# SohirMaskey/raincast-gnn

Hardware: AMD Instinct MI355X
Metric: training graphs/s (24h_mixed GNN, full train step) (higher is better)
Workload: dtype f32 (split-bf16x3 GEMM products, fp32 accumulate); 1 GPU; cfg2: 24h_mixed, 32 graphs x 500 stations, k=10, 4 GINE layers, D=128; global_batch=32, graphs_per_gpu=32, nodes_per_gpu=16000, edges_per_gpu=176000, parallelism=dp1, hip_graph=True, station_order=locality, allreduce_in_graph=False, allreduce_overlap=False, head_fold=True

## Files before the change

include/gine_hip.h:

```cpp
#ifndef GINE_HIP_H_
#define GINE_HIP_H_

#include <stddef.h>
#include <stdint.h>

#ifdef __cplusplus
extern "C" {
#endif

#define GINE_ABI_VERSION 10

#define GINE_OK 0
#define GINE_ERR_INVALID 1
#define GINE_ERR_DIM 2
#define GINE_ERR_WORKSPACE 3
#define GINE_ERR_TOO_LARGE 4
#define GINE_ERR_HIP_BASE 1000

int gine_abi_version(void);
const char* gine_status_string(int status);

int gine_graph_workspace_bytes(int64_t num_nodes, int64_t num_edges, size_t* bytes);
int gine_graph_build(const int64_t* edge_index, const float* edge_attr, int64_t num_nodes,
                     int64_t num_edges, int32_t* in_rowptr, int32_t* in_src, float* in_attr,
                     int32_t* out_rowptr, int32_t* out_dst, float* out_attr, int32_t* d_error,
                     void* workspace, size_t workspace_bytes, void* stream);
int gine_graph_same_edges(const int64_t* edge_index_a, const int64_t* edge_index_b,
                          const float* edge_attr_a, const float* edge_attr_b, int64_t num_edges,
                          int32_t* differ, void* stream);
int gine_graph_build_ek(const int64_t* edge_index, const float* edge_attr, int64_t num_nodes,
                        int64_t num_edges, int32_t edge_dim, int32_t* in_rowptr,
                        int32_t* in_src, float* in_attr, int32_t* out_rowptr, int32_t* out_dst,
                        float* out_attr, int32_t* out_eid, int32_t* d_error, void* workspace,
                        size_t workspace_bytes, void* stream);
int gine_graph_same_edges_ek(const int64_t* edge_index_a, const int64_t* edge_index_b,
                             const float* edge_attr_a, const float* edge_attr_b,
                             int64_t num_edges, int32_t edge_dim, int32_t* differ, void* stream);
int gine_host_device_ptr(void* host_ptr, void** device_ptr);

#define GINE_MP_LIN_MULADD 2
int gine_mp_fwd(const float* x, const int32_t* in_rowptr, const int32_t* in_src,
                const float* in_attr, const float* lin_w, const float* lin_b, const float* eps,
                float* z, int64_t num_nodes, int32_t channels, int32_t flags, void* stream);

#define GINE_MP_BWD_SELF 1
int gine_mp_bwd_num_partials(int64_t num_nodes, int32_t channels, int32_t* num_partials);
int gine_mp_bwd(const float* dz, const float* x, const int32_t* out_rowptr,
                const int32_t* out_dst, const float* out_attr, const float* lin_w,
                const float* lin_b, const float* eps, const float* dres, float* dx,
                double* partials, int64_t num_nodes, int32_t channels, int32_t flags,
                void* stream);
int gine_mp_bwd_finalize(const double* partials, int32_t num_partials, int32_t channels,
                         float* dlin_w, float* dlin_b, float* deps, void* stream);
int gine_mp_bwd_side(const float* dz, const float* x, const int32_t* out_rowptr,
                     const int32_t* out_dst, const float* out_attr, const float* lin_w,
                     const float* lin_b, const float* eps, const float* dres, float* dx,
                     double* partials, int64_t num_nodes, int32_t channels, int32_t flags,
                     const float* wg_slab, int32_t wg_chunks, int32_t mlp_channels, float* dw1,
                     float* db1, float* dw2, float* db2, void* stream);

#define GINE_MP_MAX_EDGE_DIM 8
int gine_mp_fwd_ek(const float* x, const int32_t* in_rowptr, const int32_t* in_src,
                   const float* in_attr, const float* lin_w, const float* lin_b,
                   const float* eps, float* z, int64_t num_nodes, int64_t num_edges,
                   int32_t channels, int32_t edge_dim, void* stream);
int gine_mp_bwd_ek_num_partials(int64_t num_nodes, int32_t channels, int32_t edge_dim,
                                int32_t* num_partials);
int gine_mp_bwd_ek(const float* dz, const float* x, const int32_t* out_rowptr,
                   const int32_t* out_dst, const float* out_attr, const int32_t* out_eid,
                   const float* lin_w, const float* lin_b, const float* eps, const float* dres,
                   float* dx, float* dea, double* partials, int64_t num_nodes,
                   int64_t num_edges, int32_t channels, int32_t edge_dim, int32_t flags,
                   void* stream);
int gine_mp_bwd_ek_finalize(const double* partials, int32_t num_partials, int32_t channels,
                            int32_t edge_dim, float* dlin_w, float* dlin_b, float* deps,
                            void* stream);

#define GINE_WINDOW_LDS_BYTES (80 * 1024)
typedef struct gine_window_plan {
  const int32_t* tile_begin;
  const int32_t* win_lo;
  const int32_t* win_rows;
  int32_t num_tiles;
  int32_t slice_channels;
  int32_t max_rows, max_edges, max_nodes;
  const int16_t* slot;
  const int32_t* edge_begin;
} gine_window_plan;
int gine_graph_plan_windows(const int32_t* rowptr, const int32_t* nbr, int64_t num_nodes,
                            int32_t max_rows, int32_t max_nodes, int32_t max_edges,
                            int32_t* tile_begin, int32_t* win_lo, int32_t* win_rows,
                            int32_t* num_tiles, int32_t* maxima);
int gine_graph_plan_window_slots(const int32_t* rowptr, const int32_t* tile_begin,
                                 int32_t num_tiles, int16_t* slot);
int gine_graph_order_locality(const int32_t* rowptr, const int32_t* nbr, int64_t num_nodes,
                              int32_t* order);
int gine_mp_fwd_win(const float* x, const int32_t* in_rowptr, const int32_t* in_src,
                    const float* in_attr, const float* lin_w, const float* lin_b,
                    const float* eps, float* z, int64_t num_nodes, int32_t channels,
                    int32_t flags, const gine_window_plan* plan, void* stream);
int gine_mp_bwd_win(const float* dz, const float* x, const int32_t* out_rowptr,
                    const int32_t* out_dst, const float* out_attr, const float* lin_w,
                    const float* lin_b, const float* eps, const float* dres, float* dx,
                    double* partials, int64_t num_nodes, int32_t channels, int32_t flags,
                    const gine_window_plan* plan, void* stream);
int gine_mp_bwd_win_side(const float* dz, const float* x, const int32_t* out_rowptr,
                         const int32_t* out_dst, const float* out_attr, const float* lin_w,
                         const float* lin_b, const float* eps, const float* dres, float* dx,
                         double* partials, int64_t num_nodes, int32_t channels, int32_t flags,
                         const gine_window_plan* plan, const float* wg_slab, int32_t wg_chunks,
                         int32_t mlp_channels, float* dw1, float* db1, float* dw2, float* db2,
                         void* stream);
int gine_mp_bwd_win_mlp_wgrad(const float* dz, const float* x, const int32_t* out_rowptr,
                              const int32_t* out_dst, const float* out_attr,
                              const float* lin_w, const float* lin_b, const float* eps,
                              const float* dres, float* dx, double* partials,
                              int64_t num_nodes, int32_t channels, int32_t flags,
                              const gine_window_plan* plan, const float* dy, const float* y,
                              const uint8_t* mask, const float* a1, const float* bn_save,
                              const float* dbn, const float* coef, const float* z, float* slab,
                              int32_t epilogue, void* stream);
int gine_mp_bwd_win_finalize(const double* partials, int32_t num_tiles, int32_t channels,
                             int32_t slice_channels, float* dlin_w, float* dlin_b,
                             float* deps, void* stream);

#define GINE_GRAD_JOB_MP 1
#define GINE_GRAD_JOB_SLAB 2
#define GINE_GRAD_MAX_JOBS 12
typedef struct gine_grad_job {
  int32_t kind;
  int32_t rows;
  int32_t channels;
  int32_t eps_cols;
  int32_t nz;
  int32_t pad_;
  const void* src;
  int64_t cstride, zstride;
  int64_t per[4];
  int64_t wsize[4];
  float bscale[4];
  float* w[4];
  float* b[4];
} gine_grad_job;
int gine_grad_finalize_batch(const gine_grad_job* jobs, int32_t num_jobs, void* stream);
int gine_head_bwd_grad_job(int64_t num_nodes, int32_t channels, int32_t kind, const float* slab,
                           float* dw, float* db, gine_grad_job* job);
int gine_chain_wgrad_grad_job(int64_t num_nodes, int32_t hidden, int32_t in_features,
                              const float* slab, float bias_scale, float* dwp2, float* dbp2,
                              float* dwr0, float* dbr0, float* dwr1, float* dbr1, float* dwdr,
                              float* dbdr, gine_grad_job* job);
int gine_deepset_bwd_grad_job(int64_t num_nodes, int32_t in_features, int32_t hidden,
                              const float* slab, float* dw1, float* db1, gine_grad_job* job);

#define GINE_EPI_NONE 0
#define GINE_EPI_RELU 1
#define GINE_EPI_RESIDUAL_RELU 2

int gine_mlp_num_partials(int64_t num_nodes, int32_t channels, int32_t* num_partials);
int gine_mlp_fwd1(const float* z, const float* w1, const float* b1, float* a1, double* partials,
                  int64_t num_nodes, int32_t channels, void* stream);
int gine_bn_fwd_finalize(const double* partials, int32_t num_partials, const float* gamma,
                         const float* beta, float* running_mean, float* running_var,
                         int64_t* num_batches_tracked, float* bn_save, int64_t num_nodes,
                         int32_t channels, float momentum, float bn_eps, int32_t training,
                         int32_t update_running, void* stream);
int gine_mlp_fwd2(const float* a1, const float* bn_save, const float* w2, const float* b2,
                  const float* x, float* y, uint8_t* mask, int64_t num_nodes, int32_t channels,
                  int32_t epilogue, void* stream);

#define GINE_MP_FUSED_MAX_DEGREE 32
int gine_mp_fwd_mlp1(const float* x, const int32_t* in_rowptr, const int32_t* in_src,
                     const float* in_attr, const float* lin_w, const float* lin_b,
                     const float* eps, const float* w1, const float* b1, float* z, float* a1,
                     double* partials, int64_t num_nodes, int32_t channels,
                     int32_t max_in_degree, int32_t flags, void* stream);

int gine_bn_acc_words(int32_t channels, int64_t* words);
int gine_bn_acc_barrier_failures_index(int32_t channels, int64_t* index);
int gine_mlp_bwd2_acc(const float* dy, const float* y, const uint8_t* mask, const float* a1,
                      const float* bn_save, const float* w2, float* dbn, double* partials,
                      int64_t* bn_acc, int64_t num_nodes, int32_t channels, int32_t epilogue,
                      void* stream);
int gine_mlp_bwd1_bn(const float* dbn, const float* a1, const float* bn_save, int64_t* bn_acc,
                     const float* gamma, float* dgamma, float* dbeta, float* coef,
                     const float* w1, float* dz, int64_t num_nodes, int32_t channels,
                     void* stream);
int gine_mlp_bwd_layer_ok(int64_t num_nodes, int32_t channels, int32_t* ok);
int gine_mlp_bwd_layer(const float* dy, const float* y, const uint8_t* mask, const float* a1,
                       const float* bn_save, const float* w2, float* dbn, int64_t* bn_acc,
                       const float* gamma, float* dgamma, float* dbeta, float* coef,
                       const float* w1, float* dz, int64_t num_nodes, int32_t channels,
                       int32_t epilogue, void* stream);
int gine_testing_bwd_layer_extra_workgroups(int32_t extra);
int gine_mlp_fwd1_acc(const float* z, const float* w1, const float* b1, float* a1,
                      double* partials, int64_t* bn_acc, int64_t num_nodes, int32_t channels,
                      void* stream);
int gine_mp_fwd_mlp1_acc(const float* x, const int32_t* in_rowptr, const int32_t* in_src,
                         const float* in_attr, const float* lin_w, const float* lin_b,
                         const float* eps, const float* w1, const float* b1, float* z,
                         float* a1, double* partials, int64_t* bn_acc, int64_t num_nodes,
                         int32_t channels, int32_t max_in_degree, int32_t flags, void* stream);
int gine_mp_fwd_layer_ok(int64_t num_nodes, int32_t channels, int32_t max_in_degree, int32_t* ok);
int gine_testing_layer_extra_workgroups(int32_t extra);
int gine_testing_sum_32(const float* in, float* out, int32_t waves, int32_t mode, void* stream);
typedef struct gine_layer_head {
  const float* weight;
  const float* bias;
  float* raw;
  float* pred;
  const float* y_target;
  uint32_t* count_parts;
  int32_t kind;
} gine_layer_head;
int gine_mp_fwd_layer(const float* x, const int32_t* in_rowptr, const int32_t* in_src,
                      const float* in_attr, const float* lin_w, const float* lin_b,
                      const float* eps, const float* w1, const float* b1, float* z, float* a1,
                      int64_t* bn_acc, const float* gamma, const float* beta,
                      float* running_mean, float* running_var, int64_t* num_batches_tracked,
                      float* bn_save, float momentum, float bn_eps, int32_t update_running,
                      const float* w2, const float* b2, float* y, uint8_t* mask,
                      int64_t num_nodes, int32_t channels, int32_t max_in_degree, int32_t flags,
                      int32_t epilogue, const int32_t* tile_windows, int32_t window_rows,
                      const gine_layer_head* head, void* stream);
int gine_mp_fwd_layer_eval(const float* x, const int32_t* in_rowptr, const int32_t* in_src,
                           const float* in_attr, const float* lin_w, const float* lin_b,
                           const float* eps, const float* w1, const float* b1,
                           const float* gamma, const float* beta, const float* running_mean,
                           const float* running_var, float bn_eps, const float* w2,
                           const float* b2, float* y, int64_t num_nodes, int32_t channels,
                           int32_t max_in_degree, int32_t flags, int32_t epilogue,
                           const gine_layer_head* head, int32_t max_workgroups, void* stream);
int gine_mp_fwd_layer_eval_deep(const float* x, const int32_t* in_rowptr, const int32_t* in_src,
                                const float* in_attr, const float* lin_w, const float* lin_b,
                                const float* eps, const float* w1, const float* b1,
                                const float* gamma, const float* beta,
                                const float* running_mean, const float* running_var,
                                float bn_eps, const float* w2, const float* b2, float* y,
                                int64_t num_nodes, int32_t channels, int32_t max_in_degree,
                                int32_t flags, int32_t epilogue, const gine_layer_head* head,
                                int32_t max_workgroups, void* stream);
int gine_graph_plan_layer_windows(const int32_t* in_rowptr, const int32_t* in_src,
                                  int64_t num_nodes, int32_t* tile_windows, int32_t* maxima,
                                  void* stream);
int gine_mp_fwd_layer_windows_fit(int32_t window_rows, int32_t max_in_degree, int32_t* ok);
int gine_mlp_fwd2_bn(const float* a1, int64_t* bn_acc, const float* gamma, const float* beta,
                     float* running_mean, float* running_var, int64_t* num_batches_tracked,
                     float* bn_save, float momentum, float bn_eps, int32_t update_running,
                     const float* w2, const float* b2, const float* x, float* y,
                     uint8_t* mask, int64_t num_nodes, int32_t channels, int32_t epilogue,
                     void* stream);

int gine_mlp_bwd2(const float* dy, const float* y, const uint8_t* mask, const float* a1,
                  const float* bn_save, const float* w2, float* dbn, double* partials,
                  int64_t num_nodes, int32_t channels, int32_t epilogue, void* stream);
int gine_bn_bwd_finalize(const double* partials, int32_t num_partials, const float* gamma,
                         const float* bn_save, float* dgamma, float* dbeta, float* coef,
                         int64_t num_nodes, int32_t channels, int32_t training, void* stream);
int gine_mlp_bwd1(const float* dbn, const float* a1, const float* bn_save, const float* coef,
                  const float* w1, float* dz, int64_t num_nodes, int32_t channels,
                  void* stream);
int gine_mlp_wgrad_num_chunks(int64_t num_nodes, int32_t channels, int32_t* num_chunks);
int gine_mlp_wgrad(const float* dy, const float* y, const uint8_t* mask, const float* a1,
                   const float* bn_save, const float* dbn, const float* coef, const float* z,
                   float* slab, float* dw1, float* db1, float* dw2, float* db2,
                   int64_t num_nodes, int32_t channels, int32_t epilogue, void* stream);

int gine_mlp_bwd1_wgrad(const float* dy, const float* y, const uint8_t* mask, const float* a1,
                        const float* bn_save, const float* dbn, const float* coef,
                        const float* z, const float* w1, float* dz, float* slab, float* dw1,
                        float* db1, float* dw2, float* db2, int64_t num_nodes,
                        int32_t channels, int32_t epilogue, void* stream);

int gine_adamw_step(float* param, const float* grad, float* exp_avg, float* exp_avg_sq,
                    float* step, int64_t n, float lr, float beta1, float beta2, float eps,
                    float weight_decay, void* stream);
int gine_adamw_state_floats(int64_t* floats);

#define GINE_LOSS_NORMAL 0
#define GINE_LOSS_MIXED_NORMAL 1
#define GINE_LOSS_MIXED 2
#define GINE_LOSS_MIXED_U 3
int gine_crps_num_partials(int64_t num_nodes, int32_t* num_partials);
int gine_crps_fwd(const float* pred, const float* y, int64_t num_nodes, int32_t kind, double u,
                  double xi, double c, double t, double* dpred, double* partials,
                  double* loss_out, double* count_out, uint32_t* ticket, void* stream);
int gine_crps_bwd(const double* dpred, const double* count, const double* gloss,
                  int64_t num_nodes, int32_t kind, float* grad_pred, void* stream);
#define GINE_COUNT_PARTS 64
int gine_count_valid(const float* y, int64_t num_nodes, uint32_t* count_parts, void* stream);
int gine_crps_fwd_grad(const float* pred, const float* y, int64_t num_nodes, int32_t kind,
                       double u, double xi, double c, double t, double* dpred, double* partials,
                       double* loss_out, double* count_out, uint32_t* ticket,
                       const uint32_t* count_parts, float* grad_unit, void* stream);
int gine_crps_head_slab_floats(int64_t num_nodes, int32_t channels, int32_t kind,
                               size_t* floats);
int gine_crps_head_fwd_grad(const float* pred, const float* y, int64_t num_nodes, int32_t kind,
                            double u, double xi, double c, double t, double* dpred,
                            double* partials, double* loss_out, double* count_out,
                            uint32_t* ticket, const uint32_t* count_parts, float* grad_unit,
                            const float* raw, const float* h, const float* w, int32_t channels,
                            float* dh, float* head_slab, void* stream);
int gine_crps_head_grad_job(int64_t num_nodes, int32_t channels, int32_t kind,
                            const float* head_slab, float* dw, float* db, gine_grad_job* job);

#define GINE_FORECAST_UPPER 1
int gine_forecast_prob(const float* pred, int64_t num_nodes, int32_t kind, double u, double xi,
                       double c, const double* x, int32_t num_x, int32_t flags, double* out,
                       void* stream);
int gine_forecast_quantile(const float* pred, int64_t num_nodes, int32_t kind, double u,
                           double xi, double c, const double* level, int32_t num_levels,
                           int32_t flags, double* out, void* stream);
int gine_forecast_score_partials(int64_t num_nodes, int32_t num_x, size_t* count);
int gine_forecast_score(const float* pred, const float* y, int64_t num_nodes, int32_t kind,
                        double u, double xi, double c, const double* x, int32_t num_x,
                        double* crps_rows, double* pit_lo, double* pit_hi, double* brier,
                        double* valid, double* partials, uint32_t* ticket, void* stream);

int gine_linear_wgrad_num_chunks(int64_t rows, int32_t out_features, int32_t in_features,
                                 int32_t* num_chunks);
int gine_linear_wgrad(const float* dy, const float* x, int64_t rows, int32_t out_features,
                      int32_t in_features, float* slab, float* dw, float* db, float bias_scale,
                      void* stream);

int gine_deepset_mask_bytes(int64_t num_nodes, int32_t members, int32_t hidden, size_t* bytes);
int gine_deepset_mask_layout(int64_t num_nodes, int32_t hidden, int32_t* nodes_per_half);
int gine_deepset_fwd(const float* ens, const float* w1, const float* b1, float* r,
                     uint16_t* mask, int64_t num_nodes, int32_t members, int32_t in_features,
                     int32_t hidden, void* stream);
int gine_deepset_fwd_fold2(const float* ens, const float* w1, const float* b1, float* r,
                           uint16_t* mask, int64_t num_nodes, int32_t members,
                           int32_t in_features, int32_t hidden, const float* wr1,
                           const float* br1, const float* wdr, const float* bdr, float* wfold,
                           int32_t x_features, const float* wr0, const float* br0,
                           const float* wp2, const float* bp2, float* wfold2, void* stream);
int gine_deepset_bwd_num_partials(int64_t num_nodes, int32_t hidden, int32_t* num_partials);
int gine_deepset_bwd(const float* ens, const uint16_t* mask, const float* dr, float* slab,
                     float* dw1, float* db1, int64_t num_nodes, int32_t members,
                     int32_t in_features, int32_t hidden, void* stream);

int gine_head_fwd(const float* h, const float* w, const float* b, float* raw, float* pred,
                  int64_t num_nodes, int32_t channels, int32_t kind, void* stream);
int gine_head_fwd_count(const float* h, const float* w, const float* b, float* raw,
                        float* pred, int64_t num_nodes, int32_t channels, int32_t kind,
                        const float* y, uint32_t* count_parts, void* stream);
int gine_head_bwd_slab_floats(int64_t num_nodes, int32_t channels, int32_t kind,
                              size_t* floats);
int gine_head_bwd(const float* grad_pred, const float* raw, const float* h, const float* w,
                  float* dh, float* slab, float* dw, float* db, int64_t num_nodes,
                  int32_t channels, int32_t kind, void* stream);
int gine_head_bwd_reduce(const float* slab, float* dw, float* db, int64_t num_nodes,
                         int32_t channels, int32_t kind, void* stream);

int gine_chain_bwd_slab_floats(int64_t num_nodes, int32_t hidden, int32_t in_features,
                               size_t* floats);
int gine_chain_fwd_folded2(const float* r, const float* x, const float* wfold,
                           const float* wfold2, float* u, float* h0, int64_t num_nodes,
                           int32_t hidden, int32_t in_features, void* stream);
int gine_chain_bwd_folded2(const float* dh0, const float* u, const float* wfold,
                           const float* wfold2, float* dt, float* dr, int64_t num_nodes,
                           int32_t hidden, int32_t in_features, void* stream);
int gine_chain_wgrad_folded2(const float* dh0, const float* x, const float* r, const float* u,
                             const float* dt, float* slab, float* gfold, float* g2fold,
                             int64_t num_nodes, int32_t hidden, int32_t in_features,
                             void* stream);
int gine_chain_wgrad_folded2_grad_job(int64_t num_nodes, int32_t hidden, int32_t in_features,
                                      const float* slab, float* gfold, float* g2fold,
                                      gine_grad_job* job);
int gine_chain_unfold_grads2(const float* gfold, const float* wr1, const float* br1,
                             const float* wdr, float* dwdr, float* dbdr, float* dwr1,
                             float* dbr1, const float* g2fold, const float* wp2,
                             const float* bp2, const float* wr0, float* dwr0, float* dbr0,
                             float* dwp2, float* dbp2, float members, int32_t hidden,
                             int32_t in_features, void* stream);
int gine_chain_fwd(const float* r, const float* x, const float* wp2, const float* bp2,
                   float bias_scale, const float* wr0, const float* br0, const float* wr1,
                   const float* br1, const float* wdr, const float* bdr, float* s, float* u,
                   float* e, float* h0, int64_t num_nodes, int32_t hidden,
                   int32_t in_features, void* stream);
int gine_chain_bwd(const float* dh0, const float* x, const float* r, const float* s,
                   const float* u, const float* e, const float* wp2, const float* wr0,
                   const float* wr1, const float* wdr, float* de, float* dt, float* ds,
                   float* dr, float* slab, float* dwp2, float* dbp2, float bias_scale,
                   float* dwr0, float* dbr0, float* dwr1, float* dbr1, float* dwdr,
                   float* dbdr, int64_t num_nodes, int32_t hidden, int32_t in_features,
                   void* stream);
int gine_chain_wgrad(const float* dh0, const float* x, const float* r, const float* s,
                     const float* u, const float* e, const float* de, const float* dt,
                     const float* ds, float* slab, float* dwp2, float* dbp2, float bias_scale,
                     float* dwr0, float* dbr0, float* dwr1, float* dbr1, float* dwdr,
                     float* dbdr, int64_t num_nodes, int32_t hidden, int32_t in_features,
                     void* stream);


int gine_copy_f4(const void* src, void* dst, int64_t bytes, void* stream);
int gine_probe_chain(int32_t variant, int32_t reps, int32_t blocks, float* sink,
                     long long* ticks, void* stream);

#ifdef __cplusplus
}
#endif

#endif
```

raincast-gnn_amd/csrc/gine_chain.hip:

```cpp
#include "gine_common.hpp"
#include "gine_slab.hpp"
#include "gine_wgrad.hpp"
#include "gine_chainfold.hpp"

#include <algorithm>

namespace gine {
namespace {

typedef float floatx16 __attribute__((ext_vector_type(16)));

constexpr int kRowTile = 32;

#ifdef GINE_CHAIN_PROFILE
__device__ long long g_chain_prof[1024][16];
#define CHAIN_MARK(i)                                                          \
  do {                                                                         \
    if (threadIdx.x == 0 && blockIdx.x < 1024)                                 \
      g_chain_prof[blockIdx.x][i] = (long long)__builtin_amdgcn_s_memtime();  \
  } while (0)
#define CHAIN_RT(i)                                                            \
  do {                                                                         \
    if (threadIdx.x == 0 && blockIdx.x < 1024)                                 \
      g_chain_prof[blockIdx.x][i] = (long long)__builtin_amdgcn_s_memrealtime(); \
  } while (0)
#else
#define CHAIN_MARK(i) do {} while (0)
#define CHAIN_RT(i) do {} while (0)
#endif

enum ChainKind { CH_F2D, CH_B2D, CH_F1, CH_F2, CH_B1, CH_B2 };

struct ChainArgs {
  const float* in;
  const float* x;
  const float* aux;
  const float* w1;
  const float* b1;
  const float* w2;
  const float* b2;
  float* out1;
  float* out2;
  float bias1_scale;
  int F;
  const float* w3;
  float* out3;
  const float* b3;
};

__device__ __forceinline__ floatx16 zero16() {
  floatx16 v;
#pragma unroll
  for (int i = 0; i < 16; ++i) v[i] = 0.f;
  return v;
}

template <int K>
__device__ __forceinline__ floatx16 tile_mma(const float* sA, int lda, const float (&bf)[K / 2],
                                             int c32, int h) {
  constexpr int KS = K / 2;
  floatx16 acc = zero16();
  const float* arow = sA + c32 * lda + h * KS;
#pragma unroll
  for (int q = 0; q < KS / 4; ++q) {
    const float4 a4 = *reinterpret_cast<const float4*>(&arow[4 * q]);
    acc = __builtin_amdgcn_mfma_f32_32x32x2f32(a4.x, bf[4 * q], acc, 0, 0, 0);
    acc = __builtin_amdgcn_mfma_f32_32x32x2f32(a4.y, bf[4 * q + 1], acc, 0, 0, 0);
    acc = __builtin_amdgcn_mfma_f32_32x32x2f32(a4.z, bf[4 * q + 2], acc, 0, 0, 0);
    acc = __builtin_amdgcn_mfma_f32_32x32x2f32(a4.w, bf[4 * q + 3], acc, 0, 0, 0);
  }
  return acc;
}

template <int K>
__device__ __forceinline__ void frag_t(float (&bf)[K / 2], const float* W, int ldw, int col,
                                       int h) {
  constexpr int KS = K / 2;
#pragma unroll
  for (int s = 0; s < KS; ++s) bf[s] = W[(size_t)col * ldw + h * KS + s];
}
template <int K>
__device__ __forceinline__ void frag_t4(float (&bf)[K / 2], const float* W, int ldw, int col,
                                        int h) {
  constexpr int KS = K / 2;
  const float4* row = reinterpret_cast<const float4*>(W + (size_t)col * ldw + h * KS);
#pragma unroll
  for (int s = 0; s < KS / 4; ++s) {
    const float4 v = row[s];
    bf[4 * s] = v.x;
    bf[4 * s + 1] = v.y;
    bf[4 * s + 2] = v.z;
    bf[4 * s + 3] = v.w;
  }
}
template <int K>
__device__ __forceinline__ void frag_n(float (&bf)[K / 2], const float* W, int ldw, int coff,
                                       int col, int h) {
  constexpr int KS = K / 2;
#pragma unroll
  for (int s = 0; s < KS; ++s) bf[s] = W[(size_t)(h * KS + s) * ldw + coff + col];
}
template <int FP, int D>
__device__ __forceinline__ void frag_dimred(float (&bf)[(FP + D) / 2], const float* W, int F,
                                            int col, int h) {
  constexpr int KS = (FP + D) / 2;
  const int ldw = F + D;
#pragma unroll
  for (int s = 0; s < KS; ++s) {
    const int k = h * KS + s;
    const int c = k < F ? k : (k < FP ? 0 : k - FP + F);
    const float v = W[(size_t)col * ldw + c];
    bf[s] = (k >= F && k < FP) ? 0.f : v;
  }
}
template <int FP, int D>
__device__ __forceinline__ void frag_dimred_t(float (&bf)[(FP + D) / 2], const float* WT, int F,
                                              int col, int h) {
  constexpr int KS = (FP + D) / 2;
#pragma unroll
  for (int s = 0; s < KS; ++s) {
    const int k = h * KS + s;
    const int c = k < F ? k : (k < FP ? 0 : k - FP + F);
    const float v = WT[(size_t)c * D + col];
    bf[s] = (k >= F && k < FP) ? 0.f : v;
  }
}

struct TileRange {
  int first, end, step;
};
__device__ __forceinline__ TileRange tile_range(int num_tiles, int nb) {
  const int xcd = blockIdx.x % kNumXcd, pos = blockIdx.x / kNumXcd;
  const int here = nb / kNumXcd + (xcd < nb % kNumXcd ? 1 : 0);
  const int span = (num_tiles + kNumXcd - 1) / kNumXcd;
  const int b = xcd * span;
  return TileRange{b + pos, min(num_tiles, b + span), here};
}

template <int D, int FP, int KIND>
__global__ __launch_bounds__(2 * D) void k_chain(ChainArgs a, int64_t N, int num_tiles) {
  constexpr int NT = 2 * D;
  constexpr int D4 = D / 4;
  constexpr int LDA = D + 4;
  constexpr bool kDimRed = KIND == CH_F2;
  constexpr int K2 = kDimRed ? FP + D : D;
  constexpr int LDB = K2 + 4;
  constexpr int BOFF = kDimRed ? FP : 0;
  constexpr int ITEMS = kRowTile * D4 / NT;
  constexpr int RSTEP = NT / D4;
  constexpr int XITEMS = (kRowTile * FP + NT - 1) / NT;
  constexpr bool kF2D = KIND == CH_F2D, kB2D = KIND == CH_B2D;
  constexpr bool kMask = KIND == CH_B1 || kB2D;
  constexpr bool kX = kDimRed || kF2D;
  constexpr int LDC = FP + D + 4;
  __shared__ __attribute__((aligned(16))) float sA[kRowTile * LDA];
  __shared__ __attribute__((aligned(16))) float sB[kF2D ? 4 : kRowTile * LDB];
  __shared__ __attribute__((aligned(16))) float sC[kF2D ? kRowTile * LDC : 4];

  const int wave = threadIdx.x / kWave, lane = threadIdx.x % kWave;
  const int h = lane >> 5, c32 = lane & 31;
  const int col = wave * 32 + c32;
  const int q_me = threadIdx.x % D4, r_me = threadIdx.x / D4;
  CHAIN_RT(11);
  CHAIN_MARK(0);
  const int nb = gridDim.x;

  float bf1[D / 2], bf2[K2 / 2];
  const bool w16 =
      ((reinterpret_cast<uintptr_t>(a.w1) | reinterpret_cast<uintptr_t>(a.w2)) & 15) == 0;
  if constexpr (KIND == CH_F1) {
    if (w16) {
      frag_t4<D>(bf1, a.w1, D, col, h);
      frag_t4<D>(bf2, a.w2, D, col, h);
    } else {
      frag_t<D>(bf1, a.w1, D, col, h);
      frag_t<D>(bf2, a.w2, D, col, h);
    }
  } else if constexpr (kF2D) {
    if (w16) frag_t4<D>(bf1, a.w1, D, col, h);
    else frag_t<D>(bf1, a.w1, D, col, h);
  } else if constexpr (KIND == CH_F2) {
    frag_t<D>(bf1, a.w1, D, col, h);
  } else if constexpr (kMask) {
    frag_n<D>(bf1, a.w1, a.F + D, a.F, col, h);
  } else if constexpr (KIND == CH_B2) {
    frag_n<D>(bf1, a.w1, D, 0, col, h);
  }
  if constexpr (KIND == CH_F2) {
    frag_dimred<FP, D>(bf2, a.w2, a.F, col, h);
  } else if constexpr (KIND == CH_B1 || KIND == CH_B2 || kB2D) {
    frag_n<D>(bf2, a.w2, D, 0, col, h);
  }
  float bf3[kF2D ? (FP + D) / 2 : 1];
  if constexpr (kF2D) frag_dimred_t<FP, D>(bf3, a.w3, a.F, col, h);
  float bias1 = 0.f, bias2 = 0.f, bias3 = 0.f;
  if constexpr (KIND == CH_F1 || KIND == CH_F2 || kF2D) bias1 = a.b1[col] * a.bias1_scale;
  if constexpr (KIND == CH_F1 || kDimRed) bias2 = a.b2[col];
  if constexpr (kF2D) bias3 = a.b3[col];
  CHAIN_MARK(1);

  auto load_tile = [&](int tile, float4 (&raw)[ITEMS], float (&xr)[XITEMS]) {
    const int64_t n0 = (int64_t)tile * kRowTile;
#pragma unroll
    for (int i = 0; i < ITEMS; ++i) {
      int64_t n = n0 + r_me + i * RSTEP;
      n = n < N ? n : N - 1;
      raw[i] = reinterpret_cast<const float4*>(a.in + n * D)[q_me];
    }
    if constexpr (kX) {
#pragma unroll
      for (int i = 0; i < XITEMS; ++i) {
        const int idx = threadIdx.x + i * NT;
        const int r = idx / FP, c = idx % FP;
        int64_t n = n0 + r;
        n = n < N ? n : N - 1;
        xr[i] = a.x[n * a.F + min(c, a.F - 1)];
      }
    }
  };

  const TileRange tr = tile_range(num_tiles, nb);
  float4 raw[ITEMS];
  float xr[XITEMS];
  if (tr.first < tr.end) load_tile(tr.first, raw, xr);
  int kt = 0;
  for (int tile = tr.first; tile < tr.end; tile += tr.step, ++kt) {
    const int64_t n0 = (int64_t)tile * kRowTile;
    float ep[16];
    if constexpr (kMask) {
#pragma unroll
      for (int r = 0; r < 16; ++r) {
        int64_t n = n0 + (r & 3) + 8 * (r >> 2) + 4 * h;
        n = n < N ? n : N - 1;
        ep[r] = a.aux[n * D + col];
      }
    }
    __syncthreads();
#pragma unroll
    for (int i = 0; i < ITEMS; ++i) {
      const int r = r_me + i * RSTEP;
      const float4 v = (n0 + r < N) ? raw[i] : f4_zero();
      float* dst = &sA[r * LDA + 4 * q_me];
      *reinterpret_cast<float4*>(dst) = v;
    }
    if constexpr (kX) {
      float* sx = kF2D ? sC : sB;
      constexpr int LDX = kF2D ? LDC : LDB;
#pragma unroll
      for (int i = 0; i < XITEMS; ++i) {
        const int idx = threadIdx.x + i * NT;
        if (idx < kRowTile * FP) sx[(idx / FP) * LDX + idx % FP] = idx % FP < a.F ? xr[i] : 0.f;
      }
    }
    __syncthreads();
    if (kt < 2) CHAIN_MARK(2 + 4 * kt);
    if (tile + tr.step < tr.end) load_tile(tile + tr.step, raw, xr);

    floatx16 acc;
    acc = tile_mma<D>(sA, LDA, bf1, c32, h);
#pragma unroll
    for (int r = 0; r < 16; ++r) {
      const int rr = (r & 3) + 8 * (r >> 2) + 4 * h;
      const int64_t n = n0 + rr;
      float v = acc[r] + bias1;
      if constexpr (kB2D) v = ep[r] > 0.f ? acc[r] : 0.f;
      if constexpr (kF2D) {
        v = relu_nan(v);
        sC[rr * LDC + FP + col] = v;
      } else {
        sB[rr * LDB + BOFF + col] = v;
      }
      if (n < N) a.out1[n * D + col] = v;
    }
    if (kt < 2) CHAIN_MARK(3 + 4 * kt);
    __syncthreads();
    if (kt < 2) CHAIN_MARK(4 + 4 * kt);

    if constexpr (!kF2D) {
      acc = tile_mma<K2>(sB, LDB, bf2, c32, h);
#pragma unroll
      for (int r = 0; r < 16; ++r) {
        const int rr = (r & 3) + 8 * (r >> 2) + 4 * h;
        const int64_t n = n0 + rr;
        float v = acc[r] + bias2;
        if constexpr (KIND == CH_F1) v = relu_nan(v);
        if constexpr (KIND == CH_B1) v = ep[r] > 0.f ? v : 0.f;
        if (n < N) a.out2[n * D + col] = v;
      }
    } else {
      acc = tile_mma<FP + D>(sC, LDC, bf3, c32, h);
#pragma unroll
      for (int r = 0; r < 16; ++r) {
        const int64_t n = n0 + (r & 3) + 8 * (r >> 2) + 4 * h;
        if (n < N) a.out3[n * D + col] = acc[r] + bias3;
      }
    }
    if (kt < 2) CHAIN_MARK(5 + 4 * kt);
  }
  CHAIN_MARK(10);
  CHAIN_RT(12);
}

inline int chain_grid(int64_t N) {
  const int64_t tiles = ceil_div(N, kRowTile);
  return (int)std::max<int64_t>(1, std::min<int64_t>(tiles, kNumCu));
}

template <int D, int FP, int KIND>
int launch_chain(const ChainArgs& a, int64_t N, hipStream_t s) {
  const int tiles = (int)ceil_div(N, kRowTile);
  hipLaunchKernelGGL((k_chain<D, FP, KIND>), dim3(chain_grid(N)), dim3(2 * D), 0, s, a, N,
                     tiles);
  GINE_LAUNCH_STATUS();
  return GINE_OK;
}

template <int NZ>
struct ChainWgradSrc {
  static constexpr int kZ = NZ;
  const float* p[NZ];
  const float* q[NZ];
  const float* x;
  int D, F;
  struct Raw {
    float4 v;
  };
  struct Col {
    float keep[4];
  };
  template <int Z> __device__ int i_dim(int) const { return Z == 0 ? F + D : D; }
  template <int Z> __device__ Col p_col(int) const { return Col{{1.f, 1.f, 1.f, 1.f}}; }
  template <int Z> __device__ Col q_col(int q4) const {
    Col c{{1.f, 1.f, 1.f, 1.f}};
    if constexpr (Z == 0) {
#pragma unroll
      for (int j = 0; j < 4; ++j) c.keep[j] = 4 * q4 + j < F + D ? 1.f : 0.f;
    }
    return c;
  }
  template <int Z> __device__ Raw p_load(int64_t n, int q4) const {
    return Raw{reinterpret_cast<const float4*>(p[Z] + n * D)[q4]};
  }
  template <int Z> __device__ Raw q_load(int64_t n, int q4) const {
    if constexpr (Z == 0) {
      const int I = F + D;
      float v[4];
#pragma unroll
      for (int j = 0; j < 4; ++j) {
        const int c = min(4 * q4 + j, I - 1);
        const float* src = c < F ? x + n * F + c : q[0] + n * D + (c - F);
        v[j] = *src;
      }
      return Raw{make_float4(v[0], v[1], v[2], v[3])};
    } else {
      return Raw{reinterpret_cast<const float4*>(q[Z] + n * D)[q4]};
    }
  }
  template <int Z> __device__ float4 p_xform(const Raw& r, const Col&) const { return r.v; }
  template <int Z> __device__ float4 q_xform(const Raw& r, const Col& c) const {
    if constexpr (Z == 0)
      return make_float4(c.keep[0] != 0.f ? r.v.x : 0.f, c.keep[1] != 0.f ? r.v.y : 0.f,
                         c.keep[2] != 0.f ? r.v.z : 0.f, c.keep[3] != 0.f ? r.v.w : 0.f);
    return r.v;
  }
};

struct ChainWgradOut {
  float* w[4];
  float* b[4];
  int D, F;
  float bscale3;
  __device__ void operator()(int z, int64_t e, double v) const {
    const int64_t I = z == 0 ? F + D : D;
    const int64_t ws = (int64_t)D * I;
    if (e < ws) {
      w[z][e] = (float)v;
    } else if (e < ws + D && b[z] != nullptr) {
      b[z][e - ws] = (float)(z == 3 ? v * (double)bscale3 : v);
    }
  }
};

struct ChainWgradShape {
  WgPlan plan;
  int nz;
  int tiles;
  size_t per;
  size_t zstride() const { return per * plan.chunks; }
  size_t slab_floats() const { return nz * zstride(); }
};
inline ChainWgradShape chain_wgrad_shape(int64_t N, int D, int F, int nz) {
  const int to = (int)ceil_div(D, 64);
  ChainWgradShape s;
  s.nz = nz;
  s.tiles = to * (int)ceil_div(F + D, kWgTI) + (nz - 1) * to * (int)ceil_div(D, kWgTI);
  s.plan = wg_plan(N, D, F + D, nz, 64, s.tiles);
  s.per = (size_t)D * (D + F) + D;
  return s;
}

void chain_slab_job(const ChainWgradShape& sh, int D, int F, const float* slab, float bscale3,
                    float* const* w, float* const* b, gine_grad_job* job) {
  *job = gine_grad_job{};
  job->kind = GINE_GRAD_JOB_SLAB;
  job->src = slab;
  job->rows = sh.plan.chunks;
  job->cstride = (int64_t)sh.per;
  job->zstride = (int64_t)sh.zstride();
  job->nz = sh.nz;
  for (int z = 0; z < sh.nz; ++z) {
    const int64_t ws = (int64_t)D * (z == 0 ? F + D : D);
    job->per[z] = ws + D;
    job->wsize[z] = ws;
    job->w[z] = w[z];
    job->b[z] = b[z];
    job->bscale[z] = z == 3 ? bscale3 : 1.0f;
  }
}

inline bool chain_dims_ok(int D, int F) { return (D == 64 || D == 128) && F >= 1 && F <= 64; }

#define GINE_CHAIN_DISPATCH(D_, F_, CALL)                          \
  do {                                                             \
    if ((D_) == 64) {                                              \
      if ((F_) <= 40) { CALL(64, 40); } else { CALL(64, 64); }     \
    } else {                                                       \
      if ((F_) <= 40) { CALL(128, 40); } else { CALL(128, 64); }   \
    }                                                              \
  } while (0)

struct UnfoldJob {
  const float *gf, *w1, *b1, *wdr;
  float *dwdr, *dbdr, *dw1, *db1;
  int F;
  float bscale;
};

template <int D>
__global__ __launch_bounds__(2 * D) void k_chain_unfold(UnfoldJob j0, UnfoldJob j1) {
  constexpr int NT = 2 * D, LDA = D + 4, T = D / 32, TT = T * T;
  constexpr int SI = 32 * D / NT, XI = 32 * 64 / NT;
  __shared__ __attribute__((aligned(16))) float sA[32 * LDA];
  __shared__ float sR[T * kSR];
  __shared__ float svec[D];
  const bool second = (int)blockIdx.x >= 2 * TT;
  const UnfoldJob J{second ? j1.gf : j0.gf,     second ? j1.w1 : j0.w1,
                    second ? j1.b1 : j0.b1,     second ? j1.wdr : j0.wdr,
                    second ? j1.dwdr : j0.dwdr, second ? j1.dbdr : j0.dbdr,
                    second ? j1.dw1 : j0.dw1,   second ? j1.db1 : j0.db1,
                    second ? j1.F : j0.F,       second ? j1.bscale : j0.bscale};
  const int blk = (int)blockIdx.x - (second ? 2 * TT : 0);
  const float* __restrict__ gf = J.gf;
  const int F = J.F;
  const int LW = F + D;
  const float* g = gf + (size_t)D * LW;
  const int w = threadIdx.x / kWave, lane = threadIdx.x % kWave;
  const int h = lane >> 5, c32 = lane & 31;
  const bool e_cols = blk < TT;
  const int t = e_cols ? blk : blk - TT;
  const int r0 = 32 * (t / T), c0 = 32 * (t % T);
  float bf[16], st[SI];
  if (e_cols) {
#pragma unroll
    for (int s = 0; s < 16; ++s) bf[s] = J.w1[(size_t)(c0 + c32) * D + w * 32 + h * 16 + s];
#pragma unroll
    for (int i = 0; i < SI; ++i) {
      const int idx = threadIdx.x + i * NT;
      st[i] = gf[(size_t)(r0 + idx / D) * LW + F + idx % D];
    }
    if (c0 == 0) {
      if (F > 0) {
        float xv[XI];
#pragma unroll
        for (int i = 0; i < XI; ++i) {
          const int idx = min(threadIdx.x + i * NT, 32 * F - 1);
          xv[i] = gf[(size_t)(r0 + idx / F) * LW + idx % F];
        }
#pragma unroll
        for (int i = 0; i < XI; ++i) {
          const int idx = threadIdx.x + i * NT;
          if (idx < 32 * F) J.dwdr[(size_t)(r0 + idx / F) * LW + idx % F] = xv[i];
        }
      }
      if (threadIdx.x < 32 && J.dbdr != nullptr) J.dbdr[r0 + threadIdx.x] = g[r0 + threadIdx.x];
    }
#pragma unroll
    for (int i = 0; i < SI; ++i) {
      const int idx = threadIdx.x + i * NT;
      sA[(idx / D) * LDA + idx % D] = st[i];
    }
  } else {
#pragma unroll
    for (int s = 0; s < 16; ++s)
      bf[s] = gf[(size_t)(w * 32 + h * 16 + s) * LW + F + c0 + c32];
#pragma unroll
    for (int i = 0; i < SI; ++i) {
      const int idx = threadIdx.x + i * NT;
      st[i] = J.wdr[(size_t)(idx / 32) * LW + F + r0 + idx % 32];
    }
    const float gv = threadIdx.x < D ? g[threadIdx.x] : 0.f;
#pragma unroll
    for (int i = 0; i < SI; ++i) {
      const int idx = threadIdx.x + i * NT;
      sA[(idx % 32) * LDA + idx / 32] = st[i];
    }
    if (threadIdx.x < D) svec[threadIdx.x] = gv;
  }
  __syncthreads();
  ksplit_tile<D>(sA, bf, sR, c32, h);
  if (!e_cols && c0 == 0) {
    const float v = rows_dot<D>(sA, svec);
    constexpr int TPR = NT / 32;
    if (threadIdx.x % TPR == 0 && J.db1 != nullptr) J.db1[r0 + threadIdx.x / TPR] = v * J.bscale;
  }
  __syncthreads();
#pragma unroll
  for (int i = 0; i < 1024 / NT; ++i) {
    const int o = threadIdx.x + i * NT, rr = o / 32, cc = o % 32;
    const float v = ksplit_sum<D>(sR, rr, cc);
    if (e_cols)
      J.dwdr[(size_t)(r0 + rr) * LW + F + c0 + cc] =
          fmaf(g[r0 + rr], J.b1[c0 + cc] * J.bscale, v);
    else
      J.dw1[(size_t)(r0 + rr) * D + c0 + cc] = v;
  }
}

int launch_unfold(int D, const UnfoldJob& j0, const UnfoldJob& j1, hipStream_t st) {
  if (D == 64)
    hipLaunchKernelGGL((k_chain_unfold<64>), dim3(2 * 2 * 4), dim3(128), 0, st, j0, j1);
  else
    hipLaunchKernelGGL((k_chain_unfold<128>), dim3(2 * 2 * 16), dim3(256), 0, st, j0, j1);
  GINE_LAUNCH_STATUS();
  return GINE_OK;
}

}
}

using namespace gine;

extern "C" int gine_chain_bwd_slab_floats(int64_t num_nodes, int32_t hidden,
                                          int32_t in_features, size_t* floats) {
  if (!floats || num_nodes < 0) return GINE_ERR_INVALID;
  if (!chain_dims_ok(hidden, in_features)) return GINE_ERR_DIM;
  *floats = std::max(chain_wgrad_shape(num_nodes, hidden, in_features, 2).slab_floats(),
                     chain_wgrad_shape(num_nodes, hidden, in_features, 4).slab_floats());
  return GINE_OK;
}

extern "C" int gine_chain_fwd_folded2(const float* r, const float* x, const float* wfold,
                                      const float* wfold2, float* u, float* h0,
                                      int64_t num_nodes, int32_t hidden, int32_t in_features,
                                      void* stream) {
  if (!chain_dims_ok(hidden, in_features)) return GINE_ERR_DIM;
  if (num_nodes < 0) return GINE_ERR_INVALID;
  if (num_nodes >= (int64_t(1) << 31)) return GINE_ERR_TOO_LARGE;
  if (num_nodes == 0) return GINE_OK;
  if (!r || !x || !wfold || !wfold2 || !u || !h0) return GINE_ERR_INVALID;
  hipStream_t st = as_stream(stream);
  const int D = hidden, F = in_features;
  const float* bfold = wfold + (size_t)D * (F + D);
  ChainArgs f{r, x, nullptr, wfold2, wfold2 + (size_t)D * D, nullptr, nullptr, u, nullptr,
              1.f, F};
  f.w3 = bfold + D;
  f.b3 = bfold;
  f.out3 = h0;
  int rc = GINE_OK;
#define CALL_F(DD, FF) rc = launch_chain<DD, FF, CH_F2D>(f, num_nodes, st)
  GINE_CHAIN_DISPATCH(D, F, CALL_F);
#undef CALL_F
  return rc;
}

extern "C" int gine_chain_bwd_folded2(const float* dh0, const float* u, const float* wfold,
                                      const float* wfold2, float* dt, float* dr,
                                      int64_t num_nodes, int32_t hidden, int32_t in_features,
                                      void* stream) {
  if (!chain_dims_ok(hidden, in_features)) return GINE_ERR_DIM;
  if (num_nodes <= 0) return GINE_ERR_INVALID;
  if (num_nodes >= (int64_t(1) << 31)) return GINE_ERR_TOO_LARGE;
  if (!dh0 || !u || !wfold || !wfold2 || !dt || !dr) return GINE_ERR_INVALID;
  hipStream_t st = as_stream(stream);
  const int F = in_features;
  const ChainArgs b{dh0, nullptr, u, wfold, nullptr, wfold2, nullptr, dt, dr, 1.f, F};
  int rc = GINE_OK;
#define CALL_B(DD, FF) rc = launch_chain<DD, FF, CH_B2D>(b, num_nodes, st)
  GINE_CHAIN_DISPATCH(hidden, F, CALL_B);
#undef CALL_B
  return rc;
}

extern "C" int gine_chain_wgrad_folded2(const float* dh0, const float* x, const float* r,
                                        const float* u, const float* dt, float* slab,
                                        float* gfold, float* g2fold, int64_t num_nodes,
                                        int32_t hidden, int32_t in_features, void* stream) {
  if (!chain_dims_ok(hidden, in_features)) return GINE_ERR_DIM;
  if (num_nodes <= 0) return GINE_ERR_INVALID;
  if (!dh0 || !x || !r || !u || !dt || !slab) return GINE_ERR_INVALID;
  const bool reduce = gfold || g2fold;
  if (reduce && (!gfold || !g2fold)) return GINE_ERR_INVALID;
  hipStream_t st = as_stream(stream);
  const int D = hidden, F = in_features;
  const ChainWgradShape sh = chain_wgrad_shape(num_nodes, D, F, 2);
  const ChainWgradSrc<2> src{{dh0, dt}, {u, r}, x, D, F};
  int rc = launch_wgrad_engine<64>(src, num_nodes, D, D + F, sh.tiles, sh.plan, sh.zstride(),
                                   sh.per, slab, st);
  if (rc != GINE_OK || !reduce) return rc;
  return launch_slab_sum(slab, sh.plan.chunks, (int64_t)sh.per, sh.per, sh.zstride(), sh.nz,
                         ChainWgradOut{{gfold, g2fold, nullptr, nullptr},
                                       {gfold + (size_t)D * (F + D), g2fold + (size_t)D * D,
                                        nullptr, nullptr},
                                       D, F, 1.f},
                         st);
}

extern "C" int gine_chain_wgrad_folded2_grad_job(int64_t num_nodes, int32_t hidden,
                                                 int32_t in_features, const float* slab,
                                                 float* gfold, float* g2fold,
                                                 gine_grad_job* job) {
  if (!chain_dims_ok(hidden, in_features)) return GINE_ERR_DIM;
  if (num_nodes <= 0 || !slab || !gfold || !g2fold || !job) return GINE_ERR_INVALID;
  const int D = hidden, F = in_features;
  float* w[2] = {gfold, g2fold};
  float* b[2] = {gfold + (size_t)D * (D + F), g2fold + (size_t)D * D};
  chain_slab_job(chain_wgrad_shape(num_nodes, D, F, 2), D, F, slab, 1.f, w, b, job);
  return GINE_OK;
}

extern "C" int gine_chain_unfold_grads2(const float* gfold, const float* wr1, const float* br1,
                                        const float* wdr, float* dwdr, float* dbdr, float* dwr1,
                                        float* dbr1, const float* g2fold, const float* wp2,
                                        const float* bp2, const float* wr0, float* dwr0,
                                        float* dbr0, float* dwp2, float* dbp2, float members,
                                        int32_t hidden, int32_t in_features, void* stream) {
  if (!chain_dims_ok(hidden, in_features)) return GINE_ERR_DIM;
  if (!gfold || !wr1 || !br1 || !wdr || !dwdr || !dwr1) return GINE_ERR_INVALID;
  if (!g2fold || !wp2 || !bp2 || !wr0 || !dwr0 || !dwp2) return GINE_ERR_INVALID;
  return launch_unfold(hidden,
                       UnfoldJob{gfold, wr1, br1, wdr, dwdr, dbdr, dwr1, dbr1, in_features, 1.f},
                       UnfoldJob{g2fold, wp2, bp2, wr0, dwr0, dbr0, dwp2, dbp2, 0, members},
                       as_stream(stream));
}

extern "C" int gine_chain_fwd(const float* r, const float* x, const float* wp2, const float* bp2,
                              float bias_scale, const float* wr0, const float* br0,
                              const float* wr1, const float* br1, const float* wdr,
                              const float* bdr, float* s, float* u, float* e, float* h0,
                              int64_t num_nodes, int32_t hidden, int32_t in_features,
                              void* stream) {
  if (!chain_dims_ok(hidden, in_features)) return GINE_ERR_DIM;
  if (num_nodes < 0) return GINE_ERR_INVALID;
  if (num_nodes >= (int64_t(1) << 31)) return GINE_ERR_TOO_LARGE;
  if (num_nodes == 0) return GINE_OK;
  if (!r || !x || !wp2 || !bp2 || !wr0 || !br0 || !wr1 || !br1 || !wdr || !bdr || !s || !u ||
      !e || !h0)
    return GINE_ERR_INVALID;
  hipStream_t st = as_stream(stream);
  const ChainArgs f1{r, nullptr, nullptr, wp2, bp2, wr0, br0, s, u, bias_scale, in_features};
  const ChainArgs f2{u, x, nullptr, wr1, br1, wdr, bdr, e, h0, 1.f, in_features};
  int rc = GINE_OK;
#define CALL_F(DD, FF)                                                  \
  rc = launch_chain<DD, FF, CH_F1>(f1, num_nodes, st);                  \
  if (rc == GINE_OK) rc = launch_chain<DD, FF, CH_F2>(f2, num_nodes, st)
  GINE_CHAIN_DISPATCH(hidden, in_features, CALL_F);
#undef CALL_F
  return rc;
}

extern "C" int gine_chain_bwd(const float* dh0, const float* x, const float* r, const float* s,
                              const float* u, const float* e, const float* wp2,
                              const float* wr0, const float* wr1, const float* wdr, float* de,
                              float* dt, float* ds, float* dr, float* slab, float* dwp2,
                              float* dbp2, float bias_scale, float* dwr0, float* dbr0,
                              float* dwr1, float* dbr1, float* dwdr, float* dbdr,
                              int64_t num_nodes, int32_t hidden, int32_t in_features,
                              void* stream) {
  if (!chain_dims_ok(hidden, in_features)) return GINE_ERR_DIM;
  if (num_nodes <= 0) return GINE_ERR_INVALID;
  if (num_nodes >= (int64_t(1) << 31)) return GINE_ERR_TOO_LARGE;
  if (!dh0 || !x || !r || !s || !u || !e || !wp2 || !wr0 || !wr1 || !wdr || !de || !dt ||
      !ds || !dr)
    return GINE_ERR_INVALID;
  if (slab && (!dwp2 || !dwr0 || !dwr1 || !dwdr)) return GINE_ERR_INVALID;
  hipStream_t st = as_stream(stream);
  const int D = hidden, F = in_features;
  const ChainArgs b1{dh0, nullptr, u, wdr, nullptr, wr1, nullptr, de, dt, 1.f, F};
  const ChainArgs b2{dt, nullptr, nullptr, wr0, nullptr, wp2, nullptr, ds, dr, 1.f, F};
  int rc = GINE_OK;
#define CALL_B(DD, FF)                                                  \
  rc = launch_chain<DD, FF, CH_B1>(b1, num_nodes, st);                  \
  if (rc == GINE_OK) rc = launch_chain<DD, FF, CH_B2>(b2, num_nodes, st)
  GINE_CHAIN_DISPATCH(D, F, CALL_B);
#undef CALL_B
  if (rc != GINE_OK || !slab) return rc;
  return gine_chain_wgrad(dh0, x, r, s, u, e, de, dt, ds, slab, dwp2, dbp2, bias_scale, dwr0,
                          dbr0, dwr1, dbr1, dwdr, dbdr, num_nodes, hidden, in_features, stream);
}

extern "C" int gine_chain_wgrad(const float* dh0, const float* x, const float* r,
                                const float* s, const float* u, const float* e,
                                const float* de, const float* dt, const float* ds, float* slab,
                                float* dwp2, float* dbp2, float bias_scale, float* dwr0,
                                float* dbr0, float* dwr1, float* dbr1, float* dwdr, float* dbdr,
                                int64_t num_nodes, int32_t hidden, int32_t in_features,
                                void* stream) {
  if (!chain_dims_ok(hidden, in_features)) return GINE_ERR_DIM;
  if (num_nodes <= 0) return GINE_ERR_INVALID;
  if (!dh0 || !x || !r || !s || !u || !e || !de || !dt || !ds || !slab) return GINE_ERR_INVALID;
  const bool reduce = dwp2 || dwr0 || dwr1 || dwdr;
  if (reduce && (!dwp2 || !dwr0 || !dwr1 || !dwdr)) return GINE_ERR_INVALID;
  hipStream_t st = as_stream(stream);
  const int D = hidden, F = in_features;
  const ChainWgradShape sh = chain_wgrad_shape(num_nodes, D, F, 4);
  const ChainWgradSrc<4> src{{dh0, de, dt, ds}, {e, u, s, r}, x, D, F};
  int rc = launch_wgrad_engine<64>(src, num_nodes, D, D + F, sh.tiles, sh.plan, sh.zstride(),
                                   sh.per, slab, st);
  if (rc != GINE_OK || !reduce) return rc;
  return launch_slab_sum(slab, sh.plan.chunks, (int64_t)sh.per, sh.per, sh.zstride(), sh.nz,
                         ChainWgradOut{{dwdr, dwr1, dwr0, dwp2}, {dbdr, dbr1, dbr0, dbp2}, D,
                                       F, bias_scale},
                         st);
}

extern "C" int gine_chain_wgrad_grad_job(int64_t num_nodes, int32_t hidden, int32_t in_features,
                                         const float* slab, float bias_scale, float* dwp2,
                                         float* dbp2, float* dwr0, float* dbr0, float* dwr1,
                                         float* dbr1, float* dwdr, float* dbdr,
                                         gine_grad_job* job) {
  if (!chain_dims_ok(hidden, in_features)) return GINE_ERR_DIM;
  if (num_nodes <= 0 || !slab || !dwp2 || !dwr0 || !dwr1 || !dwdr || !job)
    return GINE_ERR_INVALID;
  float* w[4] = {dwdr, dwr1, dwr0, dwp2};
  float* b[4] = {dbdr, dbr1, dbr0, dbp2};
  chain_slab_job(chain_wgrad_shape(num_nodes, hidden, in_features, 4), hidden, in_features,
                 slab, bias_scale, w, b, job);
  return GINE_OK;
}

#ifdef GINE_CHAIN_PROFILE
extern "C" int gine_debug_chain_prof(long long* out) {
  GINE_RETURN_IF_HIP(hipDeviceSynchronize());
  GINE_RETURN_IF_HIP(hipMemcpyFromSymbol(out, HIP_SYMBOL(g_chain_prof), sizeof(g_chain_prof)));
  return GINE_OK;
}
#endif
```

raincast-gnn_amd/csrc/gine_deepset.hip:

```cpp
#include "gine_common.hpp"
#include "gine_chainfold.hpp"
#include "gine_bf16x3.hpp"

#include <algorithm>

namespace gine {
namespace {

typedef float floatx16 __attribute__((ext_vector_type(16)));

__host__ __device__ constexpr int tiles_per_group(int G, int M) { return (G * M + 15) / 16; }

#ifndef GINE_DS_BF16X3
#define GINE_DS_BF16X3 1
#endif
template <int KP>
struct DsImg {
  static constexpr int KX = (KP + 15) / 16 * 16;
  static constexpr int RS = KX + 8;
  static constexpr int PLANE = 32 * RS;
  static constexpr int FLOATS = 3 * PLANE / 2;
};
template <int KI>
struct DsBwdImg {
  static_assert(KI == 32 || KI == 64, "feature tiles");
  static constexpr int RS = 40;
  static constexpr int PLANE = KI * RS;
  static constexpr int FLOATS = 3 * PLANE / 2;
};
constexpr int ds_bwd_ki(int KP) { return KP <= 32 ? 32 : 64; }
template <int KP, bool X3, int KI>
constexpr int stager_ld() {
  if constexpr (!X3) return KP + 4;
  else if constexpr (KI == 0) return DsImg<KP>::RS;
  else return DsBwdImg<KI>::RS;
}
template <int KP, bool X3, int KI>
constexpr int stager_plane() {
  if constexpr (!X3) return 0;
  else if constexpr (KI == 0) return DsImg<KP>::PLANE;
  else return DsBwdImg<KI>::PLANE;
}

#ifdef GINE_DS_PROFILE
__device__ long long g_ds_prof[4096];
__device__ int g_ds_prof_n;
#define DS_MARK(tag)                                                          \
  do {                                                                        \
    if (blockIdx.x == 0 && threadIdx.x == 0 && g_ds_prof_n < 2040) {          \
      g_ds_prof[2 * g_ds_prof_n] = (tag);                                     \
      g_ds_prof[2 * g_ds_prof_n + 1] = (long long)__builtin_amdgcn_s_memtime(); \
      ++g_ds_prof_n;                                                          \
    }                                                                         \
  } while (0)
#else
#define DS_MARK(tag) do {} while (0)
#endif

__device__ __forceinline__ floatx16 zero16() {
  floatx16 v;
#pragma unroll
  for (int i = 0; i < 16; ++i) v[i] = 0.f;
  return v;
}

__device__ __forceinline__ int staged_row(int i) {
  return 16 * ((i >> 2) & 1) + (i & 3) + 4 * (i >> 3);
}

#ifndef GINE_DS_BRANCHLESS
#define GINE_DS_BRANCHLESS 3
#endif
template <int NT, int KP, bool PAD, bool X3 = false, int KI = 0, bool BWD = false>
struct Stager {
  static constexpr int PER = (32 * KP + NT - 1) / NT;
  static constexpr int LD = stager_ld<KP, X3, KI>();
  static constexpr int kPlane = stager_plane<KP, X3, KI>();
  static constexpr bool kBranchless = (GINE_DS_BRANCHLESS & (BWD ? 1 : 2)) != 0;
  __device__ static int dummy_slot() {
    const int r = threadIdx.x & 31, u = threadIdx.x >> 5;
    if constexpr (X3 && KI != 0) return r * LD + 32 + (u & 7);
    else if constexpr (X3) return r * LD + DsImg<KP>::KX + (u & 7);
    else return r * LD + KP + (u & 3);
  }
  int src[PER];
  int row[PER];
  int dst[PER];
  uint32_t jrow[PAD ? PER : 1];
  __device__ __forceinline__ void init(int F, int M, int G) {
#pragma unroll
    for (int i = 0; i < PER; ++i) {
      const int e = threadIdx.x + i * NT;
      const int c = e >= 16 * F ? 1 : 0;
      const int off = e - c * 16 * F;
      const int j = off / F, f = off - j * F;
      const bool has = e < 32 * F;
      src[i] = has ? c * G * M * F + off : 0;
      row[i] = has ? c * G * M + j : 0x7fffffff;
      if constexpr (X3 && KI != 0)
        dst[i] = has ? f * LD + (16 * c + j) : (kBranchless ? dummy_slot() : -1);
      else
        dst[i] = has ? (16 * c + j) * LD + f : (kBranchless ? dummy_slot() : -1);
      if constexpr (PAD) jrow[i] = has ? (uint32_t)j : 0u;
    }
  }
  __device__ __forceinline__ uint32_t load(float (&v)[PER], const float* __restrict__ ens,
                                           int64_t row0, int64_t rows_total, int F,
                                           int half_lim) const {
    const int64_t d = rows_total - row0;
    const int lim = d <= 0 ? 0 : (d > 0x7fffffff ? 0x7fffffff : (int)d);
    const float* __restrict__ base = lim > 0 ? ens + row0 * F : ens;
    uint32_t ok = 0;
#pragma unroll
    for (int i = 0; i < PER; ++i) {
      bool in = row[i] < lim;
      if constexpr (PAD) in = in && (int)jrow[i] < half_lim;
      const int off = in ? src[i] : 0;
#ifdef GINE_BOUNDS_CHECK
      const int64_t a = (base - ens) + off;
      if (a < 0 || a >= rows_total * F) {
        printf("GINE_BOUNDS_CHECK deepset Stager::load: block %d thread %d reads ens[%lld] "
               "outside [0, %lld)\n", (int)blockIdx.x, (int)threadIdx.x, (long long)a,
               (long long)(rows_total * F));
        __builtin_trap();
      }
#endif
      v[i] = base[off];
      ok |= (in ? 1u : 0u) << i;
    }
    return ok;
  }
  __device__ __forceinline__ void store(float* s_e, const float (&v)[PER], uint32_t ok) const {
    if constexpr (X3) {
      constexpr int PL = kPlane;
      uint16_t* img = reinterpret_cast<uint16_t*>(s_e);
#pragma unroll
      for (int i = 0; i < PER; i += 2) {
        const int i1 = i + 1 < PER ? i + 1 : i;
        const float a = ((ok >> i) & 1u) ? v[i] : 0.f;
        const float b = ((ok >> i1) & 1u) ? v[i1] : 0.f;
        uint32_t ph, pm, pl;
        split2(a, b, ph, pm, pl);
        if (kBranchless || dst[i] >= 0) {
          img[dst[i]] = (uint16_t)ph;
          img[PL + dst[i]] = (uint16_t)pm;
          img[2 * PL + dst[i]] = (uint16_t)pl;
        }
        if (i + 1 < PER && (kBranchless || dst[i1] >= 0)) {
          img[dst[i1]] = (uint16_t)(ph >> 16);
          img[PL + dst[i1]] = (uint16_t)(pm >> 16);
          img[2 * PL + dst[i1]] = (uint16_t)(pl >> 16);
        }
      }
    } else {
#pragma unroll
      for (int i = 0; i < PER; ++i)
        if (kBranchless || dst[i] >= 0) s_e[dst[i]] = ((ok >> i) & 1u) ? v[i] : 0.f;
    }
  }
};

template <int KP>
__device__ __forceinline__ void zero_pad(float* s_e, int F) {
  constexpr int LD = KP + 4;
  for (int i = threadIdx.x; i < 32 * (LD - F); i += blockDim.x) {
    const int r = i / (LD - F), c = F + i % (LD - F);
    s_e[r * LD + c] = 0.f;
  }
}
template <int KP>
__device__ __forceinline__ void zero_pad_x3(float* s_e, int F) {
  using I = DsImg<KP>;
  uint16_t* img = reinterpret_cast<uint16_t*>(s_e);
  const int w = I::RS - F;
  for (int i = threadIdx.x; i < 3 * 32 * w; i += blockDim.x) {
    const int pr = i / w, c = F + i % w;
    img[pr * I::RS + c] = 0;
  }
}

template <int KP>
__device__ __forceinline__ floatx16 pre_tile(const float* s_e, const float (&bf)[KP / 2],
                                             int c32, int h) {
  constexpr int LD = KP + 4;
  constexpr int KS = KP / 2;
  floatx16 acc = zero16();
  const float* arow = s_e + staged_row(c32) * LD + h * KS;
#pragma unroll
  for (int q = 0; q < KS / 4; ++q) {
    const float4 a4 = *reinterpret_cast<const float4*>(arow + 4 * q);
    acc = __builtin_amdgcn_mfma_f32_32x32x2f32(a4.x, bf[4 * q], acc, 0, 0, 0);
    acc = __builtin_amdgcn_mfma_f32_32x32x2f32(a4.y, bf[4 * q + 1], acc, 0, 0, 0);
    acc = __builtin_amdgcn_mfma_f32_32x32x2f32(a4.z, bf[4 * q + 2], acc, 0, 0, 0);
    acc = __builtin_amdgcn_mfma_f32_32x32x2f32(a4.w, bf[4 * q + 3], acc, 0, 0, 0);
  }
  return acc;
}

template <int KP>
__device__ __forceinline__ floatx16 pre_tile_x3(const float* s_e,
                                                const Bf16x3 (&wb)[DsImg<KP>::KX / 16],
                                                int c32, int h) {
  using I = DsImg<KP>;
  const uint16_t* img = reinterpret_cast<const uint16_t*>(s_e) + staged_row(c32) * I::RS + 8 * h;
  floatx16 acc = zero16();
#pragma unroll
  for (int b = 0; b < I::KX / 16; ++b) {
    Bf16x3 a;
    a.h = *reinterpret_cast<const bf16x8_t*>(img + 16 * b);
    a.m = *reinterpret_cast<const bf16x8_t*>(img + I::PLANE + 16 * b);
    a.l = *reinterpret_cast<const bf16x8_t*>(img + 2 * I::PLANE + 16 * b);
    acc = mfma_bf16x3(a, wb[b], acc);
  }
  return acc;
}
template <int KP>
__device__ __forceinline__ void load_b_x3(const float* __restrict__ w1, int col, int h, int F,
                                          Bf16x3 (&wb)[DsImg<KP>::KX / 16]) {
#pragma unroll
  for (int b = 0; b < DsImg<KP>::KX / 16; ++b) {
    float v[8];
#pragma unroll
    for (int j = 0; j < 8; ++j) {
      const int k = 16 * b + 8 * h + j;
      v[j] = k < F ? w1[(size_t)col * F + k] : 0.f;
    }
    wb[b] = split8(make_float4(v[0], v[1], v[2], v[3]), make_float4(v[4], v[5], v[6], v[7]));
  }
}
template <int KP>
__device__ __noinline__ floatx16 pre_tile_mem(const float* __restrict__ ens,
                                              const float* __restrict__ w1, int64_t row0,
                                              int64_t rows_total, int GM, int half_lim, int F,
                                              int col, int c32, int h) {
  constexpr int KS = KP / 2;
  const int tr = staged_row(c32), c = tr >> 4, j = tr & 15;
  const int64_t grow = row0 + (int64_t)c * GM + j;
  const bool valid = grow < rows_total && j < half_lim;
  floatx16 acc = zero16();
#pragma unroll 1
  for (int s = 0; s < KS; ++s) {
    const int k = h * KS + s;
    const float a = (valid && k < F) ? ens[grow * F + k] : 0.f;
    const float b = k < F ? w1[(size_t)col * F + k] : 0.f;
    acc = __builtin_amdgcn_mfma_f32_32x32x2f32(a, b, acc, 0, 0, 0);
  }
  return acc;
}

template <int KP>
__device__ __forceinline__ void load_b(const float* __restrict__ w1, int col, int h, int F,
                                       float (&bf)[KP / 2]) {
  constexpr int KS = KP / 2;
#pragma unroll
  for (int s = 0; s < KS; ++s) {
    const int k = h * KS + s;
    bf[s] = k < F ? w1[(size_t)col * F + k] : 0.f;
  }
}

struct Groups {
  int first, step, end;
  __device__ __forceinline__ Groups(int num_groups, int nb, int b = (int)blockIdx.x) {
    const int xcd = b % kNumXcd, pos = b / kNumXcd;
    const int q = nb / kNumXcd, rm = nb % kNumXcd;
    const int here = q + (xcd < rm ? 1 : 0);
    const int before = xcd * q + min(xcd, rm);
    const int lo = (int)((int64_t)num_groups * before / nb);
    end = (int)((int64_t)num_groups * (before + here) / nb);
    first = lo + pos;
    step = here;
  }
};

struct Cursor {
  int g, t;
  int64_t row;
  __device__ __forceinline__ void start(int g0, int GM) {
    g = g0;
    t = 0;
    row = (int64_t)g0 * 2 * GM;
  }
  __device__ __forceinline__ void advance(int GM, int tpg, int step) {
    if (++t == tpg) {
      t = 0;
      g += step;
      row = (int64_t)g * 2 * GM;
    } else {
      row += 16;
    }
  }
};

template <bool UNCOND, bool MASKIN, int NT, int KP, bool PAD, bool X3, int KI, bool BWD,
          class Body>
__device__ __forceinline__ void walk_tiles(const Groups& gr, int GM, int tpg,
                                           const Stager<NT, KP, PAD, X3, KI, BWD>& st,
                                           const float* __restrict__ ens, int64_t rows_total,
                                           int F, float* buf0, float* buf1,
                                           const uint16_t* __restrict__ mask_in, Body&& tile) {
  constexpr int PER = Stager<NT, KP, PAD, X3, KI, BWD>::PER;
  if (gr.first >= gr.end) return;
  const int count = ((gr.end - gr.first + gr.step - 1) / gr.step) * tpg;
  Cursor cur, pf;
  cur.start(gr.first, GM);
  pf = cur;
  auto mload = [&](const Cursor& c) -> uint32_t {
    if constexpr (MASKIN) return (uint32_t)mask_in[((int64_t)c.g * tpg + c.t) * NT + threadIdx.x];
    else return 0u;
  };
  auto sload = [&](float (&v)[PER], const Cursor& c) -> uint32_t {
    return st.load(v, ens, c.row, rows_total, F, GM - 16 * c.t);
  };
  float va[PER], vb[PER];
  uint32_t ma = 0, mb = 0, oa = 0, ob = 0;
  oa = sload(va, pf);
  ma = mload(pf);
  st.store(buf0, va, oa);
  if (count > 1) {
    pf.advance(GM, tpg, gr.step);
    ob = sload(vb, pf);
    mb = mload(pf);
  }
  pf.advance(GM, tpg, gr.step);
  __syncthreads();
  auto step = [&](int k, float (&vcur)[PER], uint32_t& mcur, uint32_t& ocur,
                  float (&vnxt)[PER], uint32_t onxt, float* bcur, float* bnxt) {
    const uint32_t bits = mcur;
    DS_MARK(0);
    if constexpr (UNCOND) {
      const bool more = k + 2 < count;
      ocur = sload(vcur, more ? pf : cur);
      mcur = mload(more ? pf : cur);
    } else if (k + 2 < count) {
      ocur = sload(vcur, pf);
      mcur = mload(pf);
    }
    DS_MARK(1);
    tile(cur, bcur, bits);
    DS_MARK(4);
    if (k + 1 < count) st.store(bnxt, vnxt, onxt);
    DS_MARK(5);
    __syncthreads();
    DS_MARK(6);
    cur.advance(GM, tpg, gr.step);
    pf.advance(GM, tpg, gr.step);
  };
  for (int k = 0; k < count; k += 2) {
    step(k, va, ma, oa, vb, ob, buf0, buf1);
    if (k + 1 < count) step(k + 1, vb, mb, ob, va, oa, buf1, buf0);
  }
}

#ifndef GINE_DS_FWD_UNCOND
#define GINE_DS_FWD_UNCOND 0
#endif
template <int H, int KP, int G, bool MASK, bool FOLD = false>
__global__ __launch_bounds__(2 * H, 4) void k_deepset_fwd(const float* __restrict__ ens,
                                                       const float* __restrict__ w1,
                                                       const float* __restrict__ b1,
                                                       float* __restrict__ r,
                                                       uint16_t* __restrict__ mask_out,
                                                       int64_t N, int M, int F,
                                                       int num_groups, FoldArgs fold,
                                                       Fold2Args fold2) {
  constexpr int NT = 2 * H;
  constexpr bool X3 = GINE_DS_BF16X3 != 0 && G == 16;
  constexpr int TILEF = X3 ? DsImg<KP>::FLOATS : 32 * (KP + 4);
  constexpr int kWalk = 2 * TILEF + 2 * G * H;
  constexpr int kFold = FOLD ? 32 * (H + 4) + (H / 32) * kSR : 0;
  __shared__ __attribute__((aligned(16))) float s_lds[kWalk > kFold ? kWalk : kFold];
  int nbw = gridDim.x, bw = blockIdx.x;
  if constexpr (FOLD) {
    constexpr int nfold = 2 * kFoldBlocks<H>;
    nbw -= nfold;
    bw -= nfold;
    if (bw < 0) {
      const int lane = threadIdx.x % kWave;
      if ((int)blockIdx.x < kFoldBlocks<H>)
        fold_tile<H>(fold, blockIdx.x, s_lds, s_lds + 32 * (H + 4), lane & 31, lane >> 5);
      else
        fold2_tile<H>(fold2, blockIdx.x - kFoldBlocks<H>, s_lds, s_lds + 32 * (H + 4),
                      lane & 31, lane >> 5);
      return;
    }
  }
  float(*s_e)[TILEF] = reinterpret_cast<float(*)[TILEF]>(s_lds);
  float* s_r = s_lds + 2 * TILEF;
  const int wave = threadIdx.x / kWave, lane = threadIdx.x % kWave;
  const int h = lane >> 5, c32 = lane & 31;
  const int col = wave * 32 + c32;
  float bf[X3 ? 1 : KP / 2];
  Bf16x3 wb[X3 ? DsImg<KP>::KX / 16 : 1];
  if constexpr (X3) {
    load_b_x3<KP>(w1, col, h, F, wb);
    zero_pad_x3<KP>(s_e[0], F);
    zero_pad_x3<KP>(s_e[1], F);
  } else {
    load_b<KP>(w1, col, h, F, bf);
    zero_pad<KP>(s_e[0], F);
    zero_pad<KP>(s_e[1], F);
  }
  const float bias = b1[col];

  Stager<NT, KP, G != 16, X3> st;
  st.init(F, M, G);
  const Groups gr(num_groups, nbw, bw);
  const int GM = G * M, tpg = tiles_per_group(G, M);
  float run = 0.f;
  float* s_mine = s_r + (G * h) * H + col;
  int node = 0, rem = M;
  walk_tiles<GINE_DS_FWD_UNCOND != 0, false>(gr, GM, tpg, st, ens, N * M, F, s_e[0], s_e[1],
                                             nullptr,
             [&](const Cursor& c, const float* buf, uint32_t) {
    if (c.t == 0) {
      node = 0;
      rem = M;
      run = 0.f;
    }
    floatx16 acc;
    if constexpr (X3) {
      acc = pre_tile_x3<KP>(buf, wb, c32, h);
      if (wave_any_nan(acc))
        acc = pre_tile_mem<KP>(ens, w1, c.row, N * M, GM, GM - 16 * c.t, F, col, c32, h);
    } else {
      acc = pre_tile<KP>(buf, bf, c32, h);
    }
    DS_MARK(2 + 0 * (int)acc[15]);
    uint32_t bits = 0;
#pragma unroll
    for (int q = 0; q < 16; ++q) {
      const float v = acc[q] + bias;
      bits |= (v > 0.f ? 1u : 0u) << q;
      run += relu_nan(v);
      if (--rem == 0) {
        if (node < G) s_mine[node * H] = run;
        run = 0.f;
        ++node;
        rem = M;
      }
    }
    DS_MARK(3 + 0 * (int)run);
    if (G * M % 16 != 0 && c.t == tpg - 1) {
      const int live = GM - 16 * c.t;
      bits &= live >= 16 ? 0xffffu : (1u << live) - 1u;
    }
    if constexpr (MASK) mask_out[((int64_t)c.g * tpg + c.t) * NT + threadIdx.x] = (uint16_t)bits;
    if (c.t == tpg - 1) {
      const int64_t n0 = (int64_t)c.g * 2 * G + G * h;
      const int64_t nvalid = N - n0;
#pragma unroll
      for (int n = 0; n < G; ++n)
        if (n < nvalid) r[(n0 + n) * H + col] = s_mine[n * H];
    }
  });
}


template <int H, int KP, int G, bool X3>
__device__ __forceinline__ bool ds_bwd_body(const float* __restrict__ ens,
                                            const uint16_t* __restrict__ mask,
                                            const float* __restrict__ dr,
                                            float* __restrict__ slab, int64_t N, int M, int F,
                                            int num_groups, float* s_lds) {
  constexpr int NT = 2 * H;
  constexpr int KI = ds_bwd_ki(KP);
  using I = DsBwdImg<KI>;
  constexpr int LD = X3 ? I::RS : KP + 4;
  constexpr int TILEF = X3 ? I::FLOATS : 32 * (KP + 4);
  constexpr int NIF = X3 ? KI / 32 : KP / 32;
  constexpr int TAIL = X3 ? 0 : KP - 32 * NIF;
  float* s_e0 = s_lds;
  float* s_e1 = s_lds + TILEF;
  float* s_dr = s_lds + 2 * TILEF;
  const int wave = threadIdx.x / kWave, lane = threadIdx.x % kWave;
  const int h = lane >> 5, c32 = lane & 31;
  const int col = wave * 32 + c32;
  if constexpr (X3) {
    uint16_t* i0 = reinterpret_cast<uint16_t*>(s_e0);
    uint16_t* i1 = reinterpret_cast<uint16_t*>(s_e1);
    const int w = (KI - F) * I::RS;
    for (int i = threadIdx.x; i < 3 * w; i += blockDim.x) {
      const int pl = i / w, e = F * I::RS + i % w;
      i0[pl * I::PLANE + e] = 0;
      i1[pl * I::PLANE + e] = 0;
    }
  } else {
    zero_pad<KP>(s_e0, F);
    zero_pad<KP>(s_e1, F);
  }

  floatx16 gw[NIF > 0 ? NIF : 1];
#pragma unroll
  for (int it = 0; it < NIF; ++it) gw[it] = zero16();
  float tw[TAIL > 0 ? TAIL : 1];
#pragma unroll
  for (int j = 0; j < TAIL; ++j) tw[j] = 0.f;
  double gb = 0.0;

  Stager<NT, KP, G != 16, X3, KI, true> st;
  st.init(F, M, G);
  const Groups gr(num_groups, gridDim.x);
  const int GM = G * M, tpg = tiles_per_group(G, M);
  const float* my_dr = s_dr + G * h * H + col;
  int node = 0, rem = M;
  walk_tiles<true, true>(gr, GM, tpg, st, ens, N * M, F, s_e0, s_e1, mask,
             [&](const Cursor& c, const float* buf, uint32_t bits) {
    if (c.t == 0) {
      const int64_t node0 = (int64_t)c.g * 2 * G;
      constexpr int kPer = 2 * G * 32 / kWave;
      float v[kPer];
#pragma unroll
      for (int j = 0; j < kPer; ++j) {
        const int i = lane + j * kWave;
        const int64_t n = node0 + (i >> 5);
        v[j] = dr[(n < N ? n : N - 1) * H + wave * 32 + (i & 31)];
      }
#pragma unroll
      for (int j = 0; j < kPer; ++j) {
        const int i = lane + j * kWave;
        s_dr[(i >> 5) * H + wave * 32 + (i & 31)] = node0 + (i >> 5) < N ? v[j] : 0.f;
      }
      node = 0;
      rem = M;
    }
    float dh[16];
    float gsum = 0.f;
#pragma unroll
    for (int q = 0; q < 16; ++q) {
      const float d = my_dr[(node < G ? node : G - 1) * H];
      const float v = ((bits >> q) & 1u) ? d : 0.f;
      dh[q] = v;
      gsum += v;
      if (--rem == 0) {
        ++node;
        rem = M;
      }
    }
    gb += (double)gsum;
    DS_MARK(2 + 0 * (int)gsum);
    if constexpr (X3) {
      const uint16_t* img = reinterpret_cast<const uint16_t*>(buf);
#pragma unroll
      for (int s8 = 0; s8 < 2; ++s8) {
        const Bf16x3 a = split8(make_float4(dh[8 * s8], dh[8 * s8 + 1], dh[8 * s8 + 2],
                                            dh[8 * s8 + 3]),
                                make_float4(dh[8 * s8 + 4], dh[8 * s8 + 5], dh[8 * s8 + 6],
                                            dh[8 * s8 + 7]));
#pragma unroll
        for (int it = 0; it < NIF; ++it) {
          const uint16_t* col = img + (32 * it + c32) * I::RS + 16 * h + 8 * s8;
          Bf16x3 b;
          b.h = *reinterpret_cast<const bf16x8_t*>(col);
          b.m = *reinterpret_cast<const bf16x8_t*>(col + I::PLANE);
          b.l = *reinterpret_cast<const bf16x8_t*>(col + 2 * I::PLANE);
          gw[it] = mfma_bf16x3(a, b, gw[it]);
        }
      }
    } else {
#pragma unroll
      for (int q = 0; q < 16; ++q) {
        const float* erow = buf + (16 * h + q) * LD;
#pragma unroll
        for (int it = 0; it < NIF; ++it)
          gw[it] = __builtin_amdgcn_mfma_f32_32x32x2f32(dh[q], erow[32 * it + c32], gw[it], 0,
                                                        0, 0);
#pragma unroll
        for (int j = 0; j < TAIL; j += 4) {
          const float4 e4 = *reinterpret_cast<const float4*>(erow + 32 * NIF + j);
          tw[j] = __builtin_fmaf(dh[q], e4.x, tw[j]);
          tw[j + 1] = __builtin_fmaf(dh[q], e4.y, tw[j + 1]);
          tw[j + 2] = __builtin_fmaf(dh[q], e4.z, tw[j + 2]);
          tw[j + 3] = __builtin_fmaf(dh[q], e4.w, tw[j + 3]);
        }
      }
    }
    DS_MARK(3 + 0 * (int)gw[0][0]);
  });
  if constexpr (X3) {
    bool bad = false;
#pragma unroll
    for (int it = 0; it < NIF; ++it) bad = bad || wave_any_nan(gw[it]);
    if (block_any(bad, reinterpret_cast<int*>(s_e0))) return false;
  }
  float* out = slab + (size_t)blockIdx.x * ((size_t)H * F + H);
#pragma unroll
  for (int it = 0; it < NIF; ++it) {
#pragma unroll
    for (int q = 0; q < 16; ++q) {
      const int o = wave * 32 + (q & 3) + 8 * (q >> 2) + 4 * h;
      if (32 * it + c32 < F) out[(size_t)o * F + 32 * it + c32] = gw[it][q];
    }
  }
#pragma unroll
  for (int j = 0; j < TAIL; ++j) {
    const float v = tw[j] + __shfl_xor(tw[j], 32, kWave);
    if (h == 0 && 32 * NIF + j < F) out[(size_t)col * F + 32 * NIF + j] = v;
  }
  gb += shfl_xor_d(gb, 32);
  if (h == 0) out[(size_t)H * F + col] = (float)gb;
  return true;
}

#ifndef GINE_DS_BWD_BF16X3
#define GINE_DS_BWD_BF16X3 0
#endif
template <int H, int KP, int G>
constexpr int ds_bwd_lds_floats() {
  constexpr int f32 = 2 * 32 * (KP + 4);
  constexpr int x3 = GINE_DS_BWD_BF16X3 ? 2 * DsBwdImg<ds_bwd_ki(KP)>::FLOATS : 0;
  return (f32 > x3 ? f32 : x3) + 2 * G * H;
}

template <int H, int KP, int G>
__global__ __launch_bounds__(2 * H) void k_deepset_bwd(const float* __restrict__ ens,
                                                       const uint16_t* __restrict__ mask,
                                                       const float* __restrict__ dr,
                                                       float* __restrict__ slab, int64_t N,
                                                       int M, int F, int num_groups) {
  __shared__ __attribute__((aligned(16))) float s_lds[ds_bwd_lds_floats<H, KP, G>()];
#if GINE_DS_BWD_BF16X3
  if (ds_bwd_body<H, KP, G, true>(ens, mask, dr, slab, N, M, F, num_groups, s_lds)) return;
  __syncthreads();
#endif
  ds_bwd_body<H, KP, G, false>(ens, mask, dr, slab, N, M, F, num_groups, s_lds);
}

__global__ __launch_bounds__(256) void k_deepset_slab_reduce(const float* __restrict__ slab,
                                                             int chunks, int64_t per,
                                                             int64_t wsize,
                                                             float* __restrict__ dw,
                                                             float* __restrict__ db) {
  __shared__ double s_part[16][17];
  const int j = threadIdx.x & 15, g = threadIdx.x >> 4;
  const int64_t e = blockIdx.x * (int64_t)16 + j;
  double acc = 0.0;
  if (e < per) {
#pragma unroll 4
    for (int c = g; c < chunks; c += 16) acc += (double)slab[(size_t)c * per + e];
  }
  s_part[g][j] = acc;
  __syncthreads();
  if (g != 0 || e >= per) return;
  double v = 0.0;
#pragma unroll
  for (int k = 0; k < 16; ++k) v += s_part[k][j];
  if (e < wsize) dw[e] = (float)v;
  else if (db) db[e - wsize] = (float)v;
}

inline int pad_fwd(int F) {
  if (F <= 16) return 16;
  if (F <= 32) return 32;
  if (F <= 40) return 40;
  if (F <= 48) return 48;
  if (F <= 64) return 64;
  return -1;
}
inline int pad_bwd(int F) {
  if (F <= 16) return 16;
  if (F <= 32) return 32;
  if (F <= 36) return 36;
  if (F <= 40) return 40;
  if (F <= 48) return 48;
  if (F <= 64) return 64;
  return -1;
}

inline bool hidden_ok(int H) { return H == 32 || H == 64 || H == 128 || H == 256; }

#ifndef GINE_DS_G8_WAVES
#define GINE_DS_G8_WAVES 1024
#endif
inline int nodes_per_half(int64_t N, int H) {
  const int64_t waves16 = ceil_div(N > 0 ? N : 1, 32) * (H / 32);
  return waves16 <= 256 ? 4 : (waves16 <= GINE_DS_G8_WAVES ? 8 : 16);
}
inline int num_groups(int64_t N, int H) {
  return (int)ceil_div(N > 0 ? N : 1, 2 * nodes_per_half(N, H));
}
inline int bwd_grid(int64_t N, int H) {
  return std::min(num_groups(N, H), H >= 128 ? 512 : 1024);
}

#define DS_FWD_KP(H_, KP_, MACRO)                         \
  switch (KP_) {                                          \
    case 16: MACRO(H_, 16); break;                        \
    case 32: MACRO(H_, 32); break;                        \
    case 40: MACRO(H_, 40); break;                        \
    case 48: MACRO(H_, 48); break;                        \
    default: MACRO(H_, 64); break;                        \
  }

#define DS_BWD_KP(H_, KP_, MACRO)                         \
  switch (KP_) {                                          \
    case 16: MACRO(H_, 16); break;                        \
    case 32: MACRO(H_, 32); break;                        \
    case 36: MACRO(H_, 36); break;                        \
    case 40: MACRO(H_, 40); break;                        \
    case 48: MACRO(H_, 48); break;                        \
    default: MACRO(H_, 64); break;                        \
  }

#define DS_DISPATCH_H(H, KP, KPSWITCH, MACRO)             \
  switch (H) {                                            \
    case 32: KPSWITCH(32, KP, MACRO); break;              \
    case 64: KPSWITCH(64, KP, MACRO); break;              \
    case 128: KPSWITCH(128, KP, MACRO); break;            \
    default: KPSWITCH(256, KP, MACRO); break;             \
  }

}
}

using namespace gine;

extern "C" int gine_deepset_mask_bytes(int64_t num_nodes, int32_t members, int32_t hidden,
                                       size_t* bytes) {
  if (!bytes || num_nodes < 0 || members <= 0 || !hidden_ok(hidden)) return GINE_ERR_INVALID;
  const int G = nodes_per_half(num_nodes, hidden);
  *bytes = num_nodes == 0 ? 0
                          : (size_t)num_groups(num_nodes, hidden) * tiles_per_group(G, members) * 2 *
                                hidden * sizeof(uint16_t);
  return GINE_OK;
}

extern "C" int gine_deepset_mask_layout(int64_t num_nodes, int32_t hidden,
                                        int32_t* nodes_per_half_out) {
  if (!nodes_per_half_out || num_nodes < 0 || !hidden_ok(hidden)) return GINE_ERR_INVALID;
  *nodes_per_half_out = nodes_per_half(num_nodes, hidden);
  return GINE_OK;
}

extern "C" int gine_deepset_fwd(const float* ens, const float* w1, const float* b1, float* r,
                                uint16_t* mask, int64_t num_nodes, int32_t members,
                                int32_t in_features, int32_t hidden, void* stream) {
  const int KP = pad_fwd(in_features);
  if (!hidden_ok(hidden) || KP < 0 || in_features <= 0) return GINE_ERR_DIM;
  if (num_nodes < 0 || members <= 0) return GINE_ERR_INVALID;
  if (num_nodes == 0) return GINE_OK;
  if (!ens || !w1 || !b1 || !r) return GINE_ERR_INVALID;
  if (num_nodes * members >= (int64_t(1) << 31)) return GINE_ERR_TOO_LARGE;
  const int groups = num_groups(num_nodes, hidden);
  const int grid = std::min(groups, 1024);
  const int G = nodes_per_half(num_nodes, hidden);
  hipStream_t s = as_stream(stream);
#define LAUNCH_FWD_M(H_, KP_, G_, MK_)                                                        \
  hipLaunchKernelGGL((k_deepset_fwd<H_, KP_, G_, MK_>), dim3(grid), dim3(2 * H_), 0, s, ens, w1, \
                     b1, r, mask, num_nodes, members, in_features, groups, FoldArgs{},       \
                     Fold2Args{})
#define LAUNCH_FWD_G(H_, KP_, G_)                             \
  do {                                                        \
    if (mask) LAUNCH_FWD_M(H_, KP_, G_, true);                \
    else LAUNCH_FWD_M(H_, KP_, G_, false);                    \
  } while (0)
#define LAUNCH_FWD(H_, KP_)                                   \
  do {                                                        \
    if (G == 4) LAUNCH_FWD_G(H_, KP_, 4);                     \
    else if (G == 8) LAUNCH_FWD_G(H_, KP_, 8);                \
    else LAUNCH_FWD_G(H_, KP_, 16);                           \
  } while (0)
  DS_DISPATCH_H(hidden, KP, DS_FWD_KP, LAUNCH_FWD);
#undef LAUNCH_FWD
#undef LAUNCH_FWD_G
#undef LAUNCH_FWD_M
  GINE_LAUNCH_STATUS();
  return GINE_OK;
}

extern "C" int gine_deepset_bwd_num_partials(int64_t num_nodes, int32_t hidden,
                                             int32_t* num_partials) {
  if (!num_partials || num_nodes < 0) return GINE_ERR_INVALID;
  if (!hidden_ok(hidden)) return GINE_ERR_DIM;
  *num_partials = bwd_grid(num_nodes, hidden);
  return GINE_OK;
}

extern "C" int gine_deepset_bwd(const float* ens, const uint16_t* mask, const float* dr,
                                float* slab, float* dw1, float* db1, int64_t num_nodes,
                                int32_t members, int32_t in_features, int32_t hidden,
                                void* stream) {
  const int KP = pad_bwd(in_features);
  if (!hidden_ok(hidden) || KP < 0 || in_features <= 0) return GINE_ERR_DIM;
  if (num_nodes < 0 || members <= 0 || !slab) return GINE_ERR_INVALID;
  if (num_nodes > 0 && (!ens || !mask || !dr)) return GINE_ERR_INVALID;
  if (num_nodes * members >= (int64_t(1) << 31)) return GINE_ERR_TOO_LARGE;
  const int groups = num_groups(num_nodes, hidden);
  const int grid = bwd_grid(num_nodes, hidden);
  const int G = nodes_per_half(num_nodes, hidden);
  const int64_t per = (int64_t)hidden * in_features + hidden;
  hipStream_t s = as_stream(stream);
  if (num_nodes == 0) {
    GINE_RETURN_IF_HIP(hipMemsetAsync(slab, 0, sizeof(float) * per * grid, s));
  } else {
#define LAUNCH_BWD_G(H_, KP_, G_)                                                             \
  hipLaunchKernelGGL((k_deepset_bwd<H_, KP_, G_>), dim3(grid), dim3(2 * H_), 0, s, ens, mask,  \
                     dr, slab, num_nodes, members, in_features, groups)
#define LAUNCH_BWD(H_, KP_)                       \
  do {                                            \
    if (G == 4) LAUNCH_BWD_G(H_, KP_, 4);         \
    else if (G == 8) LAUNCH_BWD_G(H_, KP_, 8);    \
    else LAUNCH_BWD_G(H_, KP_, 16);               \
  } while (0)
    DS_DISPATCH_H(hidden, KP, DS_BWD_KP, LAUNCH_BWD);
#undef LAUNCH_BWD
#undef LAUNCH_BWD_G
    GINE_LAUNCH_STATUS();
  }
  if (!dw1) return GINE_OK;
  hipLaunchKernelGGL(k_deepset_slab_reduce, dim3((unsigned)ceil_div(per, 16)), dim3(256), 0, s,
                     slab, grid, per, (int64_t)hidden * in_features, dw1, db1);
  GINE_LAUNCH_STATUS();
  return GINE_OK;
}

extern "C" int gine_deepset_bwd_grad_job(int64_t num_nodes, int32_t in_features, int32_t hidden,
                                         const float* slab, float* dw1, float* db1,
                                         gine_grad_job* job) {
  if (!hidden_ok(hidden) || pad_bwd(in_features) < 0 || in_features <= 0) return GINE_ERR_DIM;
  if (num_nodes < 0 || !slab || !dw1 || !job) return GINE_ERR_INVALID;
  const int64_t per = (int64_t)hidden * in_features + hidden;
  *job = gine_grad_job{};
  job->kind = GINE_GRAD_JOB_SLAB;
  job->src = slab;
  job->rows = bwd_grid(num_nodes, hidden);
  job->cstride = per;
  job->nz = 1;
  job->per[0] = per;
  job->wsize[0] = (int64_t)hidden * in_features;
  job->w[0] = dw1;
  job->b[0] = db1;
  job->bscale[0] = 1.0f;
  return GINE_OK;
}

#ifdef GINE_DS_PROFILE
extern "C" int gine_debug_ds_prof(long long* out, int* n) {
  GINE_RETURN_IF_HIP(hipDeviceSynchronize());
  GINE_RETURN_IF_HIP(hipMemcpyFromSymbol(n, HIP_SYMBOL(g_ds_prof_n), sizeof(int)));
  GINE_RETURN_IF_HIP(hipMemcpyFromSymbol(out, HIP_SYMBOL(g_ds_prof), sizeof(long long) * 4096));
  const int zero = 0;
  GINE_RETURN_IF_HIP(hipMemcpyToSymbol(HIP_SYMBOL(g_ds_prof_n), &zero, sizeof(int)));
  return GINE_OK;
}
#endif

extern "C" int gine_deepset_fwd_fold2(const float* ens, const float* w1, const float* b1,
                                      float* r, uint16_t* mask, int64_t num_nodes,
                                      int32_t members, int32_t in_features, int32_t hidden,
                                      const float* wr1, const float* br1, const float* wdr,
                                      const float* bdr, float* wfold, int32_t x_features,
                                      const float* wr0, const float* br0, const float* wp2,
                                      const float* bp2, float* wfold2, void* stream) {
  if (!wr0 || !br0 || !wp2 || !bp2 || !wfold2) return GINE_ERR_INVALID;
  const int KP = pad_fwd(in_features);
  if ((hidden != 64 && hidden != 128) || KP < 0 || in_features <= 0) return GINE_ERR_DIM;
  if (x_features < 1 || x_features > 64) return GINE_ERR_DIM;
  if (num_nodes < 0 || members <= 0) return GINE_ERR_INVALID;
  if (!wr1 || !br1 || !wdr || !bdr || !wfold) return GINE_ERR_INVALID;
  const FoldArgs fold{wr1, br1, wdr, bdr, wfold, x_features};
  const Fold2Args fold2{wr0, br0, wp2, bp2, (float)members, wfold2};
  if (num_nodes > 0 && (!ens || !w1 || !b1 || !r)) return GINE_ERR_INVALID;
  if (num_nodes * members >= (int64_t(1) << 31)) return GINE_ERR_TOO_LARGE;
  const int groups = num_groups(num_nodes, hidden);
  const int walk = num_nodes > 0 ? std::min(groups, 1024) : 0;
  const int G = nodes_per_half(num_nodes, hidden);
  const int nfold = 2 * (hidden == 64 ? kFoldBlocks<64> : kFoldBlocks<128>);
  hipStream_t s = as_stream(stream);
#define LAUNCH_FWD_F(H_, KP_, G_, MK_)                                                        \
  hipLaunchKernelGGL((k_deepset_fwd<H_, KP_, G_, MK_, true>), dim3(walk + nfold),             \
                     dim3(2 * H_), 0, s, ens, w1, b1, r, mask, num_nodes, members, in_features, \
                     groups, fold, fold2)
#define LAUNCH_FWD_G(H_, KP_, G_)                             \
  do {                                                        \
    if (mask) LAUNCH_FWD_F(H_, KP_, G_, true);                \
    else LAUNCH_FWD_F(H_, KP_, G_, false);                    \
  } while (0)
#define LAUNCH_FWD(H_, KP_)                                   \
  do {                                                        \
    if (G == 4) LAUNCH_FWD_G(H_, KP_, 4);                     \
    else if (G == 8) LAUNCH_FWD_G(H_, KP_, 8);                \
    else LAUNCH_FWD_G(H_, KP_, 16);                           \
  } while (0)
  if (hidden == 64) {
    DS_FWD_KP(64, KP, LAUNCH_FWD);
  } else {
    DS_FWD_KP(128, KP, LAUNCH_FWD);
  }
#undef LAUNCH_FWD
#undef LAUNCH_FWD_G
#undef LAUNCH_FWD_F
  GINE_LAUNCH_STATUS();
  return GINE_OK;
}
```

raincast-gnn_amd/csrc/gine_wgrad.hpp:

```cpp
#pragma once

#include "gine_common.hpp"
#include "gine_bf16x3.hpp"

#ifndef GINE_WG_VARIANT
#define GINE_WG_VARIANT 0
#endif

namespace gine {

#if (GINE_WG_VARIANT & 8) != 0
__device__ unsigned long long gine_wg_clock[4096][4];
#endif

typedef float wg_floatx16 __attribute__((ext_vector_type(16)));

constexpr int kWgRows = 64;
constexpr int kWgTI = 128;
constexpr int kWgLdQ = kWgTI + 4;
#ifndef GINE_WG_TARGET_BLOCKS
#define GINE_WG_TARGET_BLOCKS 256
#endif
constexpr int kWgTargetBlocks = GINE_WG_TARGET_BLOCKS;
constexpr int kWgMinSubtiles = 2;
#ifndef GINE_WG_WAVES64
#define GINE_WG_WAVES64 8
#endif
constexpr int kWgWaves64 = GINE_WG_WAVES64;

#ifndef GINE_WG_BF16X3
#define GINE_WG_BF16X3 1
#endif

template <int C>
struct WgImg {
  static constexpr int kPlane = C * kWgRows * 2;
  static constexpr int kBytes = 3 * kPlane;
  __device__ static __forceinline__ int off(int c, int k) {
    return c * (kWgRows * 2) + 16 * ((k >> 3) ^ ((c >> 1) & 7)) + 2 * (k & 7);
  }
};

template <int TO>
constexpr size_t wg_lds_bytes() {
  constexpr size_t f32 = sizeof(float) * kWgRows * ((TO + 4) + kWgLdQ);
  constexpr size_t x3 = (size_t)3 * kWgRows * 2 * (TO + kWgTI);
  return GINE_WG_BF16X3 ? (f32 > x3 ? f32 : x3) : f32;
}

struct WgPlan {
  int tiles_o, tiles_i, chunks, rows_per_chunk;
};

inline WgPlan wg_plan(int64_t R, int O, int I, int Z, int TO, int total_tiles = 0) {
  WgPlan p;
  p.tiles_o = (int)ceil_div(O, TO);
  p.tiles_i = (int)ceil_div(I, kWgTI);
  const int64_t subtiles = ceil_div(R > 0 ? R : 1, kWgRows);
  if (total_tiles <= 0) total_tiles = Z * p.tiles_o * p.tiles_i;
  int64_t chunks = ceil_div(kWgTargetBlocks, (int64_t)total_tiles);
  const int64_t cap = ceil_div(subtiles, kWgMinSubtiles);
  if (chunks > cap) chunks = cap;
  if (chunks < 1) chunks = 1;
  const int64_t per = ceil_div(subtiles, chunks);
  p.rows_per_chunk = (int)(per * kWgRows);
  p.chunks = (int)ceil_div(R > 0 ? R : 1, p.rows_per_chunk);
  return p;
}

template <class Src, int Z, int TO, int NW>
__device__ __forceinline__ void wgrad_body(const Src& src, int64_t R, int O, int I, int chunk,
                                           int tile, int rows_per_chunk, size_t zstride,
                                           size_t cstride, float* __restrict__ slab,
                                           float* __restrict__ sP, float* __restrict__ sQ) {
  using Raw = typename Src::Raw;
  using Col = typename Src::Col;
#if (GINE_WG_VARIANT & 8) != 0
  const int blin = blockIdx.x + gridDim.x * blockIdx.y + gridDim.x * gridDim.y * blockIdx.z;
  if (threadIdx.x == 0 && blin < 4096) {
    gine_wg_clock[blin][0] = __builtin_amdgcn_s_memtime();
    gine_wg_clock[blin][1] = __builtin_amdgcn_s_memrealtime();
  }
#endif
  constexpr int NT = 64 * NW;
  constexpr int LDP = TO + 4;
  constexpr int PQ = TO / 4;
  constexpr int PG = NT / PQ;
  constexpr int PITEMS = kWgRows / PG;
  constexpr int QQ = kWgTI / 4, QG = NT / QQ;
  constexpr int QITEMS = kWgRows / QG;
  constexpr int NJ = NW == 8 ? 1 : 2;
  constexpr int NI = (NW == 4 && TO == 128) ? 2 : 1;
  static_assert(NW == 4 || (NW == 8 && TO == 64), "engine shapes");

  const int tiles_i = (int)ceil_div(I, kWgTI);
  const int o0 = (tile / tiles_i) * TO, i0 = (tile % tiles_i) * kWgTI;
  const int wave = __builtin_amdgcn_readfirstlane(threadIdx.x / kWave);
  const int lane = threadIdx.x % kWave;
  const int h = lane >> 5, c32 = lane & 31;
  const int ob = NW == 8 ? 32 * (wave >> 2) : (TO == 128 ? 64 * (wave >> 1) : 0);
  const int ib = NW == 8 ? 32 * (wave & 3) : (TO == 128 ? 64 * (wave & 1) : 32 * wave);
  const bool bias_block = (i0 == 0);

  const int pq = threadIdx.x % PQ, pr = threadIdx.x / PQ;
  const int qq = threadIdx.x % QQ, qr = threadIdx.x / QQ;
  const bool p_ok = o0 + 4 * pq < O, q_ok = i0 + 4 * qq < I;
  const int pqa = p_ok ? o0 / 4 + pq : 0, qqa = q_ok ? i0 / 4 + qq : 0;
  const Col pc = src.template p_col<Z>(pqa);
  const Col qc = src.template q_col<Z>(qqa);

  const int64_t r_begin = (int64_t)chunk * rows_per_chunk;
  const int64_t r_end = min<int64_t>(R, r_begin + rows_per_chunk);

  wg_floatx16 acc[NJ][NI];
#pragma unroll
  for (int j = 0; j < NJ; ++j)
#pragma unroll
    for (int k = 0; k < NI; ++k)
#pragma unroll
      for (int e = 0; e < 16; ++e) acc[j][k][e] = 0.f;
  double bsum[4] = {0.0, 0.0, 0.0, 0.0};

  Raw rp[PITEMS]{}, rq[QITEMS]{};
  auto load_item = [&](int j, int64_t n0) {
    if constexpr ((GINE_WG_VARIANT & 2) != 0) return;
    if (j < PITEMS) {
      const int64_t n = n0 + pr + PG * j;
      rp[j] = src.template p_load<Z>(n < r_end ? n : r_end - 1, pqa);
    } else {
      const int k = j - PITEMS;
      const int64_t n = n0 + qr + QG * k;
      rq[k] = src.template q_load<Z>(n < r_end ? n : r_end - 1, qqa);
    }
  };
  constexpr int NITEMS = PITEMS + QITEMS;
  constexpr int SP = (kWgRows / 2) / NITEMS;
  static_assert(SP >= 2, "at most one raw load per two k-steps");

  if (r_begin < r_end) {
#pragma unroll
    for (int j = 0; j < NITEMS; ++j) load_item(j, r_begin);
  }
  for (int64_t n0 = r_begin; n0 < r_end; n0 += kWgRows) {
#pragma unroll
    for (int k = 0; k < PITEMS; ++k) {
      const int r = pr + PG * k;
      float4 v = src.template p_xform<Z>(rp[k], pc);
      if (n0 + r >= r_end || !p_ok) v = f4_zero();
      *reinterpret_cast<float4*>(&sP[r * LDP + 4 * pq]) = v;
      bsum[0] += (double)v.x;
      bsum[1] += (double)v.y;
      bsum[2] += (double)v.z;
      bsum[3] += (double)v.w;
    }
#pragma unroll
    for (int k = 0; k < QITEMS; ++k) {
      const int r = qr + QG * k;
      float4 v = src.template q_xform<Z>(rq[k], qc);
      if (n0 + r >= r_end || !q_ok) v = f4_zero();
      *reinterpret_cast<float4*>(&sQ[r * kWgLdQ + 4 * qq]) = v;
    }
    __syncthreads();
    const int64_t n1 = n0 + kWgRows;
    const float* pa = &sP[(32 * h) * LDP + ob + c32];
    const float* qb = &sQ[(32 * h) * kWgLdQ + ib + c32];
    float a[NJ], b[NI], an[NJ], bn[NI];
#pragma unroll
    for (int j = 0; j < NJ; ++j) a[j] = pa[32 * j];
#pragma unroll
    for (int k = 0; k < NI; ++k) b[k] = qb[32 * k];
#pragma unroll
    for (int s = 0; s < kWgRows / 2; ++s) {
      if (s + 1 < kWgRows / 2) {
        if constexpr ((GINE_WG_VARIANT & 16) != 0) {
#pragma unroll
          for (int j = 0; j < NJ; ++j) an[j] = a[j] * 0.5f;
#pragma unroll
          for (int k = 0; k < NI; ++k) bn[k] = b[k] * 0.5f;
        } else {
#pragma unroll
          for (int j = 0; j < NJ; ++j) an[j] = pa[(s + 1) * LDP + 32 * j];
#pragma unroll
          for (int k = 0; k < NI; ++k) bn[k] = qb[(s + 1) * kWgLdQ + 32 * k];
        }
      }
      if (s % SP == 0 && s / SP < NITEMS) load_item(s / SP, n1);
      if constexpr ((GINE_WG_VARIANT & 1) == 0) {
#pragma unroll
        for (int j = 0; j < NJ; ++j)
#pragma unroll
          for (int k = 0; k < NI; ++k)
            acc[j][k] = __builtin_amdgcn_mfma_f32_32x32x2f32(a[j], b[k], acc[j][k], 0, 0, 0);
      }
      __builtin_amdgcn_sched_barrier(0);
#pragma unroll
      for (int j = 0; j < NJ; ++j) a[j] = an[j];
#pragma unroll
      for (int k = 0; k < NI; ++k) b[k] = bn[k];
    }
    __syncthreads();
  }

  float* out = slab + (size_t)Z * zstride + (size_t)chunk * cstride;
  if constexpr ((GINE_WG_VARIANT & 4) != 0) {
    if (acc[0][0][0] != 12345.f) return;
  }
#pragma unroll
  for (int k = 0; k < NI; ++k) {
    const int i = i0 + ib + 32 * k + c32;
    if (i >= I) continue;
#pragma unroll
    for (int j = 0; j < NJ; ++j) {
#pragma unroll
      for (int r = 0; r < 16; ++r) {
        const int o = o0 + ob + 32 * j + (r & 3) + 8 * (r >> 2) + 4 * h;
        if (o < O) out[(size_t)o * I + i] = acc[j][k][r];
      }
    }
  }
#if (GINE_WG_VARIANT & 8) != 0
  if (threadIdx.x == 0 && blin < 4096) {
    gine_wg_clock[blin][2] = __builtin_amdgcn_s_memtime();
    gine_wg_clock[blin][3] = __builtin_amdgcn_s_memrealtime();
  }
#endif
  if (bias_block) {
    double* sb = reinterpret_cast<double*>(sQ);
#pragma unroll
    for (int j = 0; j < 4; ++j) sb[pr * TO + 4 * pq + j] = bsum[j];
    __syncthreads();
    if ((int)threadIdx.x < TO && o0 + (int)threadIdx.x < O) {
      double t = 0.0;
#pragma unroll 8
      for (int g = 0; g < PG; ++g) t += sb[g * TO + threadIdx.x];
      out[(size_t)O * I + o0 + threadIdx.x] = (float)t;
    }
  }
}

template <int C, int ITEMS>
__device__ __forceinline__ void wg_store_cols(char* img, int cq, int k0, const float4 (&v)[ITEMS]) {
  static_assert(ITEMS == 2 || ITEMS == 4 || ITEMS == 8, "column runs");
  using Img = WgImg<C>;
#pragma unroll
  for (int e = 0; e < 4; ++e) {
    uint32_t ph[ITEMS / 2], pm[ITEMS / 2], pl[ITEMS / 2];
#pragma unroll
    for (int k = 0; k < ITEMS; k += 2) {
      const float a = e == 0 ? v[k].x : e == 1 ? v[k].y : e == 2 ? v[k].z : v[k].w;
      const float b = e == 0 ? v[k + 1].x : e == 1 ? v[k + 1].y : e == 2 ? v[k + 1].z : v[k + 1].w;
      split2(a, b, ph[k / 2], pm[k / 2], pl[k / 2]);
    }
    const int o = Img::off(4 * cq + e, k0);
    char* d[3] = {img + o, img + Img::kPlane + o, img + 2 * Img::kPlane + o};
    const uint32_t* src[3] = {ph, pm, pl};
#pragma unroll
    for (int pl3 = 0; pl3 < 3; ++pl3) {
      if constexpr (ITEMS == 2) {
        *reinterpret_cast<uint32_t*>(d[pl3]) = src[pl3][0];
      } else if constexpr (ITEMS == 4) {
        *reinterpret_cast<uint2*>(d[pl3]) = make_uint2(src[pl3][0], src[pl3][1]);
      } else {
        *reinterpret_cast<uint4*>(d[pl3]) =
            make_uint4(src[pl3][0], src[pl3][1], src[pl3][2], src[pl3][3]);
      }
    }
  }
}

template <int C>
__device__ __forceinline__ Bf16x3 wg_col_frag(const char* img, int c, int k0) {
  using Img = WgImg<C>;
  const int o = Img::off(c, k0);
  Bf16x3 f;
  f.h = *reinterpret_cast<const bf16x8_t*>(img + o);
  f.m = *reinterpret_cast<const bf16x8_t*>(img + Img::kPlane + o);
  f.l = *reinterpret_cast<const bf16x8_t*>(img + 2 * Img::kPlane + o);
  return f;
}

template <class Src, int Z, int TO, int NW>
__device__ __forceinline__ void wgrad_body_x3(const Src& src, int64_t R, int O, int I,
                                              int chunk, int tile, int rows_per_chunk,
                                              size_t zstride, size_t cstride,
                                              float* __restrict__ slab, float* __restrict__ sP,
                                              float* __restrict__ sQ) {
  using Raw = typename Src::Raw;
  using Col = typename Src::Col;
  using IP = WgImg<TO>;
  char* imgP = reinterpret_cast<char*>(sP);
  char* imgQ = imgP + IP::kBytes;
  constexpr int NT = 64 * NW;
  constexpr int PQ = TO / 4;
  constexpr int PG = NT / PQ;
  constexpr int PITEMS = kWgRows / PG;
  constexpr int QQ = kWgTI / 4, QG = NT / QQ;
  constexpr int QITEMS = kWgRows / QG;
  constexpr int NJ = NW == 8 ? 1 : 2;
  constexpr int NI = (NW == 4 && TO == 128) ? 2 : 1;
  static_assert(NW == 4 || (NW == 8 && TO == 64), "engine shapes");

  const int tiles_i = (int)ceil_div(I, kWgTI);
  const int o0 = (tile / tiles_i) * TO, i0 = (tile % tiles_i) * kWgTI;
  const int wave = __builtin_amdgcn_readfirstlane(threadIdx.x / kWave);
  const int lane = threadIdx.x % kWave;
  const int h = lane >> 5, c32 = lane & 31;
  const int ob = NW == 8 ? 32 * (wave >> 2) : (TO == 128 ? 64 * (wave >> 1) : 0);
  const int ib = NW == 8 ? 32 * (wave & 3) : (TO == 128 ? 64 * (wave & 1) : 32 * wave);
  const bool bias_block = (i0 == 0);

  const int pq = threadIdx.x % PQ, pr = threadIdx.x / PQ;
  const int qq = threadIdx.x % QQ, qr = threadIdx.x / QQ;
  const bool p_ok = o0 + 4 * pq < O, q_ok = i0 + 4 * qq < I;
  const int pqa = p_ok ? o0 / 4 + pq : 0, qqa = q_ok ? i0 / 4 + qq : 0;
  const Col pc = src.template p_col<Z>(pqa);
  const Col qc = src.template q_col<Z>(qqa);
  static_assert(PITEMS % 2 == 0 && QITEMS % 2 == 0, "column runs of 2, 4 or 8 rows");

  const int64_t r_begin = (int64_t)chunk * rows_per_chunk;
  const int64_t r_end = min<int64_t>(R, r_begin + rows_per_chunk);

  wg_floatx16 acc[NJ][NI];
#pragma unroll
  for (int j = 0; j < NJ; ++j)
#pragma unroll
    for (int k = 0; k < NI; ++k)
#pragma unroll
      for (int e = 0; e < 16; ++e) acc[j][k][e] = 0.f;
  double bsum[4] = {0.0, 0.0, 0.0, 0.0};

  Raw rp[PITEMS]{}, rq[QITEMS]{};
  auto load_item = [&](int j, int64_t n0) {
    if (j < PITEMS) {
      const int64_t n = n0 + pr * PITEMS + j;
      rp[j] = src.template p_load<Z>(n < r_end ? n : r_end - 1, pqa);
    } else {
      const int k = j - PITEMS;
      const int64_t n = n0 + qr * QITEMS + k;
      rq[k] = src.template q_load<Z>(n < r_end ? n : r_end - 1, qqa);
    }
  };
  constexpr int NITEMS = PITEMS + QITEMS;
  constexpr int KB = kWgRows / 16;

  if (r_begin < r_end) {
#pragma unroll
    for (int j = 0; j < NITEMS; ++j) load_item(j, r_begin);
  }
  for (int64_t n0 = r_begin; n0 < r_end; n0 += kWgRows) {
    {
      float4 vp[PITEMS], vq[QITEMS];
#pragma unroll
      for (int k = 0; k < PITEMS; ++k) {
        const int r = pr * PITEMS + k;
        float4 v = src.template p_xform<Z>(rp[k], pc);
        if (n0 + r >= r_end || !p_ok) v = f4_zero();
        vp[k] = v;
        bsum[0] += (double)v.x;
        bsum[1] += (double)v.y;
        bsum[2] += (double)v.z;
        bsum[3] += (double)v.w;
      }
      wg_store_cols<TO, PITEMS>(imgP, pq, pr * PITEMS, vp);
#pragma unroll
      for (int k = 0; k < QITEMS; ++k) {
        const int r = qr * QITEMS + k;
        float4 v = src.template q_xform<Z>(rq[k], qc);
        if (n0 + r >= r_end || !q_ok) v = f4_zero();
        vq[k] = v;
      }
      wg_store_cols<kWgTI, QITEMS>(imgQ, qq, qr * QITEMS, vq);
    }
    __syncthreads();
    const int64_t n1 = n0 + kWgRows;
#pragma unroll
    for (int b = 0; b < KB; ++b) {
      const int k0 = 16 * b + 8 * h;
      Bf16x3 fa[NJ], fb[NI];
#pragma unroll
      for (int j = 0; j < NJ; ++j) fa[j] = wg_col_frag<TO>(imgP, ob + 32 * j + c32, k0);
#pragma unroll
      for (int k = 0; k < NI; ++k) fb[k] = wg_col_frag<kWgTI>(imgQ, ib + 32 * k + c32, k0);
#pragma unroll
      for (int j = 0; j < NITEMS; ++j)
        if (j % KB == b) load_item(j, n1);
#pragma unroll
      for (int j = 0; j < NJ; ++j)
#pragma unroll
        for (int k = 0; k < NI; ++k) acc[j][k] = mfma_bf16x3(fa[j], fb[k], acc[j][k]);
      __builtin_amdgcn_sched_barrier(0);
    }
    __syncthreads();
  }

  bool bad = false;
#pragma unroll
  for (int j = 0; j < NJ; ++j)
#pragma unroll
    for (int k = 0; k < NI; ++k) bad = bad || wave_any_nan(acc[j][k]);
#ifndef GINE_WG_X3_NANCHECK
#define GINE_WG_X3_NANCHECK 1
#endif
  if (GINE_WG_X3_NANCHECK && block_any(bad, reinterpret_cast<int*>(imgP))) {
    wgrad_body<Src, Z, TO, NW>(src, R, O, I, chunk, tile, rows_per_chunk, zstride, cstride,
                               slab, sP, sQ);
    return;
  }

  float* out = slab + (size_t)Z * zstride + (size_t)chunk * cstride;
#pragma unroll
  for (int k = 0; k < NI; ++k) {
    const int i = i0 + ib + 32 * k + c32;
    if (i >= I) continue;
#pragma unroll
    for (int j = 0; j < NJ; ++j) {
#pragma unroll
      for (int r = 0; r < 16; ++r) {
        const int o = o0 + ob + 32 * j + (r & 3) + 8 * (r >> 2) + 4 * h;
        if (o < O) out[(size_t)o * I + i] = acc[j][k][r];
      }
    }
  }
  if (bias_block) {
    double* sb = reinterpret_cast<double*>(imgQ);
#pragma unroll
    for (int j = 0; j < 4; ++j) sb[pr * TO + 4 * pq + j] = bsum[j];
    __syncthreads();
    if ((int)threadIdx.x < TO && o0 + (int)threadIdx.x < O) {
      double t = 0.0;
#pragma unroll 8
      for (int g = 0; g < PG; ++g) t += sb[g * TO + threadIdx.x];
      out[(size_t)O * I + o0 + threadIdx.x] = (float)t;
    }
  }
}

template <bool X3, class Src, int Z, int TO, int NW>
__device__ __forceinline__ void wg_body(const Src& src, int64_t R, int O, int I, int chunk,
                                        int tile, int rows_per_chunk, size_t zstride,
                                        size_t cstride, float* __restrict__ slab, float* sP,
                                        float* sQ) {
  if constexpr (X3)
    wgrad_body_x3<Src, Z, TO, NW>(src, R, O, I, chunk, tile, rows_per_chunk, zstride, cstride,
                                  slab, sP, sQ);
  else
    wgrad_body<Src, Z, TO, NW>(src, R, O, I, chunk, tile, rows_per_chunk, zstride, cstride,
                               slab, sP, sQ);
}

template <class Src, int Z>
__device__ __forceinline__ int wg_tiles(const Src& src, int O, int I, int TO) {
  return (int)(ceil_div(O, TO) * ceil_div(src.template i_dim<Z>(I), kWgTI));
}

template <class Src, int TO, int NW, bool X3 = GINE_WG_BF16X3 != 0>
__device__ __forceinline__ void wgrad_block(const Src& src, int64_t R, int O, int I, int chunk,
                                            int y, int rows_per_chunk, size_t zstride,
                                            size_t cstride, float* __restrict__ slab,
                                            float* sP, float* sQ) {
  const int t0 = wg_tiles<Src, 0>(src, O, I, TO);
  if (y < t0) {
    wg_body<X3, Src, 0, TO, NW>(src, R, O, src.template i_dim<0>(I), chunk, y, rows_per_chunk,
                               zstride, cstride, slab, sP, sQ);
    return;
  }
  y -= t0;
  if constexpr (Src::kZ > 1) {
    const int t1 = wg_tiles<Src, 1>(src, O, I, TO);
    if (y < t1) {
      wg_body<X3, Src, 1, TO, NW>(src, R, O, src.template i_dim<1>(I), chunk, y,
                                 rows_per_chunk, zstride, cstride, slab, sP, sQ);
      return;
    }
    y -= t1;
  }
  if constexpr (Src::kZ > 2) {
    const int t2 = wg_tiles<Src, 2>(src, O, I, TO);
    if (y < t2) {
      wg_body<X3, Src, 2, TO, NW>(src, R, O, src.template i_dim<2>(I), chunk, y,
                                 rows_per_chunk, zstride, cstride, slab, sP, sQ);
      return;
    }
    y -= t2;
  }
  if constexpr (Src::kZ > 3) {
    wg_body<X3, Src, 3, TO, NW>(src, R, O, src.template i_dim<3>(I), chunk, y, rows_per_chunk,
                               zstride, cstride, slab, sP, sQ);
  }
}

template <class Src, int TO, int NW, bool X3>
__global__ __launch_bounds__(64 * NW) void k_wgrad_engine(Src src, int64_t R, int O, int I,
                                                          int rows_per_chunk, size_t zstride,
                                                          size_t cstride,
                                                          float* __restrict__ slab,
                                                          int total_tiles) {
  constexpr size_t kBytes =
      X3 ? wg_lds_bytes<TO>() : sizeof(float) * kWgRows * ((TO + 4) + kWgLdQ);
  __shared__ __attribute__((aligned(16))) float s_eng[kBytes / sizeof(float)];
  const int lb = xcd_remap(blockIdx.x, gridDim.x);
  wgrad_block<Src, TO, NW, X3>(src, R, O, I, lb / total_tiles, lb % total_tiles,
                               rows_per_chunk, zstride, cstride, slab, s_eng,
                               s_eng + kWgRows * (TO + 4));
}

template <int TO, class Src, bool X3 = GINE_WG_BF16X3 != 0>
inline int launch_wgrad_engine(const Src& src, int64_t R, int O, int I, int total_tiles,
                               const WgPlan& p, size_t zstride, size_t cstride, float* slab,
                               hipStream_t s) {
  constexpr int NW = TO == 64 ? kWgWaves64 : 4;
  hipLaunchKernelGGL((k_wgrad_engine<Src, TO, NW, X3>), dim3(p.chunks * total_tiles),
                     dim3(64 * NW), 0, s, src, R, O, I, p.rows_per_chunk, zstride, cstride,
                     slab, total_tiles);
  GINE_LAUNCH_STATUS();
  return GINE_OK;
}

}
```

raincast-gnn_amd/raincast_gnn/_lib.py:

```python
from __future__ import annotations

import ctypes
import os
import threading

import torch

_HERE = os.path.dirname(os.path.abspath(__file__))
LIB_PATH = os.environ.get("GINE_HIP_LIB", os.path.join(_HERE, "_native", "libgine_hip.so"))

GINE_OK = 0
GINE_ERR_INVALID, GINE_ERR_DIM = 1, 2
GINE_ERR_TOO_LARGE = 4
GINE_ERR_HIP_BASE = 1000
GINE_MP_BWD_SELF = 1
GINE_MP_LIN_MULADD = 2
EPI_NONE, EPI_RELU, EPI_RESIDUAL_RELU = 0, 1, 2
LOSS_NORMAL, LOSS_MIXED_NORMAL, LOSS_MIXED, LOSS_MIXED_U = 0, 1, 2, 3
ABI_VERSION = 10
COUNT_PARTS = 64
FORECAST_UPPER = 1

_c_void_p = ctypes.c_void_p
_i32, _i64, _f32, _size = ctypes.c_int32, ctypes.c_int64, ctypes.c_float, ctypes.c_size_t
_f64 = ctypes.c_double



class WindowPlan(ctypes.Structure):
    _fields_ = [("tile_begin", _c_void_p), ("win_lo", _c_void_p), ("win_rows", _c_void_p),
                ("num_tiles", _i32), ("slice_channels", _i32), ("max_rows", _i32),
                ("max_edges", _i32), ("max_nodes", _i32), ("slot", _c_void_p),
                ("edge_begin", _c_void_p)]


_plan_p = ctypes.POINTER(WindowPlan)


class GradJob(ctypes.Structure):
    _fields_ = [("kind", _i32), ("rows", _i32), ("channels", _i32), ("eps_cols", _i32),
                ("nz", _i32), ("pad_", _i32), ("src", _c_void_p), ("cstride", _i64),
                ("zstride", _i64), ("per", _i64 * 4), ("wsize", _i64 * 4),
                ("bscale", _f32 * 4), ("w", _c_void_p * 4), ("b", _c_void_p * 4)]


class LayerHead(ctypes.Structure):
    _fields_ = [("weight", _c_void_p), ("bias", _c_void_p), ("raw", _c_void_p),
                ("pred", _c_void_p), ("y_target", _c_void_p), ("count_parts", _c_void_p),
                ("kind", _i32)]


GRAD_JOB_MP, GRAD_JOB_SLAB, GRAD_MAX_JOBS = 1, 2, 12
MP_FUSED_MAX_DEGREE = 32
MP_MAX_EDGE_DIM = 8
MP_EK_MAX_CHANNELS = 256
_job_p = ctypes.POINTER(GradJob)
WINDOW_LDS_BYTES = 80 * 1024

_SIGNATURES = {
    "gine_graph_workspace_bytes": [_i64, _i64, ctypes.POINTER(_size)],
    "gine_graph_build": [_c_void_p, _c_void_p, _i64, _i64, _c_void_p, _c_void_p, _c_void_p,
                         _c_void_p, _c_void_p, _c_void_p, _c_void_p, _c_void_p, _size, _c_void_p],
    "gine_graph_same_edges": [_c_void_p] * 4 + [_i64, _c_void_p, _c_void_p],
    "gine_host_device_ptr": [_c_void_p, ctypes.POINTER(_c_void_p)],
    "gine_graph_build_ek": [_c_void_p, _c_void_p, _i64, _i64, _i32] + [_c_void_p] * 9
                           + [_size, _c_void_p],
    "gine_graph_same_edges_ek": [_c_void_p] * 4 + [_i64, _i32, _c_void_p, _c_void_p],
    "gine_mp_fwd_ek": [_c_void_p] * 8 + [_i64, _i64, _i32, _i32, _c_void_p],
    "gine_mp_bwd_ek_num_partials": [_i64, _i32, _i32, ctypes.POINTER(_i32)],
    "gine_mp_bwd_ek": [_c_void_p] * 13 + [_i64, _i64, _i32, _i32, _i32, _c_void_p],
    "gine_mp_bwd_ek_finalize": [_c_void_p, _i32, _i32, _i32, _c_void_p, _c_void_p, _c_void_p,
                                _c_void_p],
    "gine_mp_fwd": [_c_void_p] * 8 + [_i64, _i32, _i32, _c_void_p],
    "gine_mp_bwd_num_partials": [_i64, _i32, ctypes.POINTER(_i32)],
    "gine_mp_bwd": [_c_void_p] * 11 + [_i64, _i32, _i32, _c_void_p],
    "gine_mp_bwd_side": [_c_void_p] * 11 + [_i64, _i32, _i32, _c_void_p, _i32, _i32]
                        + [_c_void_p] * 5,
    "gine_mp_bwd_finalize": [_c_void_p, _i32, _i32, _c_void_p, _c_void_p, _c_void_p, _c_void_p],
    "gine_graph_order_locality": [_c_void_p, _c_void_p, _i64, _c_void_p],
    "gine_graph_plan_windows": [_c_void_p, _c_void_p, _i64, _i32, _i32, _i32, _c_void_p,
                                _c_void_p, _c_void_p, ctypes.POINTER(_i32), _c_void_p],
    "gine_mp_fwd_win": [_c_void_p] * 8 + [_i64, _i32, _i32, _plan_p, _c_void_p],
    "gine_mp_bwd_win": [_c_void_p] * 11 + [_i64, _i32, _i32, _plan_p, _c_void_p],
    "gine_mp_bwd_win_mlp_wgrad": [_c_void_p] * 11 + [_i64, _i32, _i32, _plan_p]
                                 + [_c_void_p] * 9 + [_i32, _c_void_p],
    "gine_mp_bwd_win_side": [_c_void_p] * 11 + [_i64, _i32, _i32, _plan_p, _c_void_p, _i32,
                                                 _i32] + [_c_void_p] * 5,
    "gine_mp_bwd_win_finalize": [_c_void_p, _i32, _i32, _i32, _c_void_p, _c_void_p, _c_void_p,
                                 _c_void_p],
    "gine_grad_finalize_batch": [_job_p, _i32, _c_void_p],
    "gine_head_bwd_grad_job": [_i64, _i32, _i32, _c_void_p, _c_void_p, _c_void_p, _job_p],
    "gine_deepset_bwd_grad_job": [_i64, _i32, _i32, _c_void_p, _c_void_p, _c_void_p, _job_p],
    "gine_mlp_num_partials": [_i64, _i32, ctypes.POINTER(_i32)],
    "gine_mlp_fwd1": [_c_void_p] * 5 + [_i64, _i32, _c_void_p],
    "gine_mp_fwd_mlp1": [_c_void_p] * 12 + [_i64, _i32, _i32, _i32, _c_void_p],
    "gine_mp_fwd_mlp1_acc": [_c_void_p] * 13 + [_i64, _i32, _i32, _i32, _c_void_p],
    "gine_mp_fwd_layer_ok": [_i64, _i32, _i32, ctypes.POINTER(_i32)],
    "gine_mp_fwd_layer": [_c_void_p] * 18 + [_f32, _f32, _i32] + [_c_void_p] * 4
                         + [_i64, _i32, _i32, _i32, _i32, _c_void_p, _i32,
                            ctypes.POINTER(LayerHead), _c_void_p],
    "gine_mp_fwd_layer_eval": [_c_void_p] * 13 + [_f32] + [_c_void_p] * 3
                              + [_i64, _i32, _i32, _i32, _i32, ctypes.POINTER(LayerHead), _i32,
                                 _c_void_p],
    "gine_mp_fwd_layer_eval_deep": [_c_void_p] * 13 + [_f32] + [_c_void_p] * 3
                                   + [_i64, _i32, _i32, _i32, _i32, ctypes.POINTER(LayerHead),
                                      _i32, _c_void_p],
    "gine_graph_plan_layer_windows": [_c_void_p, _c_void_p, _i64, _c_void_p, _c_void_p,
                                      _c_void_p],
    "gine_mp_fwd_layer_windows_fit": [_i32, _i32, ctypes.POINTER(_i32)],
    "gine_mlp_fwd1_acc": [_c_void_p] * 6 + [_i64, _i32, _c_void_p],
    "gine_mlp_fwd2_bn": [_c_void_p] * 8 + [_f32, _f32, _i32] + [_c_void_p] * 5
                        + [_i64, _i32, _i32, _c_void_p],
    "gine_bn_acc_words": [_i32, _c_void_p],
    "gine_bn_acc_barrier_failures_index": [_i32, _c_void_p],
    "gine_testing_layer_extra_workgroups": [_i32],
    "gine_testing_sum_32": [_c_void_p, _c_void_p, _i32, _i32, _c_void_p],
    "gine_mlp_bwd2_acc": [_c_void_p] * 9 + [_i64, _i32, _i32, _c_void_p],
    "gine_mlp_bwd1_bn": [_c_void_p] * 10 + [_i64, _i32, _c_void_p],
    "gine_mlp_bwd_layer_ok": [_i64, _i32, ctypes.POINTER(_i32)],
    "gine_mlp_bwd_layer": [_c_void_p] * 14 + [_i64, _i32, _i32, _c_void_p],
    "gine_testing_bwd_layer_extra_workgroups": [_i32],
    "gine_bn_fwd_finalize": [_c_void_p, _i32] + [_c_void_p] * 6 + [_i64, _i32, _f32, _f32, _i32,
                                                                   _i32, _c_void_p],
    "gine_mlp_fwd2": [_c_void_p] * 7 + [_i64, _i32, _i32, _c_void_p],
    "gine_mlp_bwd2": [_c_void_p] * 8 + [_i64, _i32, _i32, _c_void_p],
    "gine_bn_bwd_finalize": [_c_void_p, _i32] + [_c_void_p] * 5 + [_i64, _i32, _i32, _c_void_p],
    "gine_mlp_bwd1": [_c_void_p] * 6 + [_i64, _i32, _c_void_p],
    "gine_mlp_wgrad_num_chunks": [_i64, _i32, ctypes.POINTER(_i32)],
    "gine_mlp_wgrad": [_c_void_p] * 13 + [_i64, _i32, _i32, _c_void_p],
    "gine_mlp_bwd1_wgrad": [_c_void_p] * 15 + [_i64, _i32, _i32, _c_void_p],
    "gine_head_bwd_reduce": [_c_void_p] * 3 + [_i64, _i32, _i32, _c_void_p],
    "gine_adamw_step": [_c_void_p] * 5 + [_i64, _f32, _f32, _f32, _f32, _f32, _c_void_p],
    "gine_crps_num_partials": [_i64, ctypes.POINTER(_i32)],
    "gine_crps_fwd": [_c_void_p, _c_void_p, _i64, _i32, _f64, _f64, _f64, _f64, _c_void_p,
                      _c_void_p, _c_void_p, _c_void_p, _c_void_p, _c_void_p],
    "gine_crps_bwd": [_c_void_p, _c_void_p, _c_void_p, _i64, _i32, _c_void_p, _c_void_p],
    "gine_count_valid": [_c_void_p, _i64, _c_void_p, _c_void_p],
    "gine_adamw_state_floats": [ctypes.POINTER(_i64)],
    "gine_crps_fwd_grad": [_c_void_p, _c_void_p, _i64, _i32, _f64, _f64, _f64, _f64]
                          + [_c_void_p] * 8,
    "gine_crps_head_slab_floats": [_i64, _i32, _i32, ctypes.POINTER(ctypes.c_size_t)],
    "gine_crps_head_fwd_grad": [_c_void_p, _c_void_p, _i64, _i32, _f64, _f64, _f64, _f64]
                               + [_c_void_p] * 10 + [_i32] + [_c_void_p] * 3,
    "gine_crps_head_grad_job": [_i64, _i32, _i32, _c_void_p, _c_void_p, _c_void_p, _job_p],
    "gine_forecast_prob": [_c_void_p, _i64, _i32, _f64, _f64, _f64, _c_void_p, _i32, _i32,
                           _c_void_p, _c_void_p],
    "gine_forecast_quantile": [_c_void_p, _i64, _i32, _f64, _f64, _f64, _c_void_p, _i32, _i32,
                               _c_void_p, _c_void_p],
    "gine_forecast_score_partials": [_i64, _i32, ctypes.POINTER(_size)],
    "gine_forecast_score": [_c_void_p, _c_void_p, _i64, _i32, _f64, _f64, _f64, _c_void_p, _i32]
                           + [_c_void_p] * 8,
    "gine_linear_wgrad_num_chunks": [_i64, _i32, _i32, ctypes.POINTER(_i32)],
    "gine_linear_wgrad": [_c_void_p, _c_void_p, _i64, _i32, _i32, _c_void_p, _c_void_p,
                          _c_void_p, _f32, _c_void_p],
    "gine_deepset_mask_bytes": [_i64, _i32, _i32, ctypes.POINTER(_size)],
    "gine_deepset_mask_layout": [_i64, _i32, ctypes.POINTER(_i32)],
    "gine_copy_f4": [_c_void_p, _c_void_p, _i64, _c_void_p],
    "gine_probe_chain": [_i32, _i32, _i32, _c_void_p, _c_void_p, _c_void_p],
    "gine_deepset_fwd":[_c_void_p, _c_void_p, _c_void_p, _c_void_p, _c_void_p, _i64, _i32,
                         _i32, _i32, _c_void_p],
    "gine_deepset_bwd_num_partials": [_i64, _i32, ctypes.POINTER(_i32)],
    "gine_deepset_bwd": [_c_void_p, _c_void_p, _c_void_p, _c_void_p, _c_void_p, _c_void_p,
                         _i64, _i32, _i32, _i32, _c_void_p],
    "gine_head_fwd": [_c_void_p] * 5 + [_i64, _i32, _i32, _c_void_p],
    "gine_head_fwd_count": [_c_void_p] * 5 + [_i64, _i32, _i32] + [_c_void_p] * 3,
    "gine_head_bwd_slab_floats": [_i64, _i32, _i32, ctypes.POINTER(_size)],
    "gine_head_bwd": [_c_void_p] * 8 + [_i64, _i32, _i32, _c_void_p],
    "gine_chain_bwd_slab_floats": [_i64, _i32, _i32, ctypes.POINTER(_size)],
    "gine_chain_fwd": [_c_void_p] * 4 + [_f32] + [_c_void_p] * 10 + [_i64, _i32, _i32,
                                                                       _c_void_p],
    "gine_chain_bwd": [_c_void_p] * 17 + [_f32] + [_c_void_p] * 6 + [_i64, _i32, _i32,
                                                                       _c_void_p],
    "gine_chain_wgrad": [_c_void_p] * 12 + [_f32] + [_c_void_p] * 6 + [_i64, _i32, _i32,
                                                                        _c_void_p],
    "gine_chain_wgrad_grad_job": [_i64, _i32, _i32, _c_void_p, _f32] + [_c_void_p] * 8
                                 + [_job_p],
    "gine_graph_plan_window_slots": [_c_void_p, _c_void_p, _i32, _c_void_p],
    "gine_deepset_fwd_fold2": [_c_void_p] * 5 + [_i64, _i32, _i32, _i32] + [_c_void_p] * 5
                              + [_i32] + [_c_void_p] * 6,
    "gine_chain_fwd_folded2": [_c_void_p] * 6 + [_i64, _i32, _i32, _c_void_p],
    "gine_chain_bwd_folded2": [_c_void_p] * 6 + [_i64, _i32, _i32, _c_void_p],
    "gine_chain_wgrad_folded2": [_c_void_p] * 8 + [_i64, _i32, _i32, _c_void_p],
    "gine_chain_wgrad_folded2_grad_job": [_i64, _i32, _i32] + [_c_void_p] * 3 + [_job_p],
    "gine_chain_unfold_grads2": [_c_void_p] * 16 + [_f32, _i32, _i32, _c_void_p],
}

EXPORTED_SYMBOLS = ("gine_abi_version", "gine_status_string") + tuple(_SIGNATURES)

_lock = threading.Lock()
_lib = None


class GineError(RuntimeError):
    """A native entry point returned a non-zero status."""


def load(path: str | None = None) -> ctypes.CDLL:
    global _lib
    with _lock:
        if _lib is not None and path is None:
            return _lib
        p = path or LIB_PATH
        if not os.path.exists(p):
            raise GineError(
                f"native GINE library not found at {p}; build it with "
                "`python -c 'import __graft_entry__ as g; g.build()'` (hipcc, gfx950)")
        lib = ctypes.CDLL(p)
        lib.gine_abi_version.restype = ctypes.c_int
        lib.gine_abi_version.argtypes = []
        lib.gine_status_string.restype = ctypes.c_char_p
        lib.gine_status_string.argtypes = [ctypes.c_int]
        for name, argtypes in _SIGNATURES.items():
            fn = getattr(lib, name)
            fn.restype = ctypes.c_int
            fn.argtypes = argtypes
        if lib.gine_abi_version() != ABI_VERSION:
            raise GineError(f"ABI mismatch: library {lib.gine_abi_version()} != {ABI_VERSION}")
        if path is None:
            _lib = lib
        return lib


def check(status: int, what: str) -> None:
    if status != GINE_OK:
        msg = load().gine_status_string(status).decode()
        raise GineError(f"{what} failed with status {status}: {msg}")


def call(name: str, *args) -> None:
    check(getattr(load(), name)(*args), name)


def ptr(t) -> int | None:
    if t is None:
        return None
    return t.data_ptr()


def stream_handle(device: torch.device) -> int:
    return torch.cuda.current_stream(device).cuda_stream


def require_device(t: torch.Tensor, what: str) -> None:
    if not t.is_cuda:
        raise GineError(
            f"{what}: the MI355X GINE engine runs on HIP devices only (got a {t.device} tensor); "
            "there is no CPU fallback")
```

raincast-gnn_amd/raincast_gnn/chain.py:

```python
from __future__ import annotations

import ctypes

import torch

from . import _lib, gradbuf
from .gradbuf import grad_out

HIDDEN = (64, 128)
MAX_FEATURES = 64


def fusable(r: torch.Tensor, x: torch.Tensor, lins) -> bool:
    return r.is_cuda and r.dtype == torch.float32 and fusable_dims(r.size(1), x, lins)


def fusable_dims(D: int, x: torch.Tensor, lins) -> bool:
    p2, r0, r1, dr = lins
    F = x.size(1)
    shapes = ((p2, D, D), (r0, D, D), (r1, D, D), (dr, F + D, D))
    return (x.is_cuda and x.dtype == torch.float32
            and D in HIDDEN and 0 < F <= MAX_FEATURES and not x.requires_grad
            and all(isinstance(m, torch.nn.Linear) and m.bias is not None
                    and m.weight.dtype == torch.float32 and m.in_features == i
                    and m.out_features == o for m, i, o in shapes))


class _ChainFn(torch.autograd.Function):
    @staticmethod
    def forward(ctx, r, x, wp2, bp2, wr0, br0, wr1, br1, wdr, bdr, members):
        r = r.contiguous()
        x = x.contiguous()
        N, D = r.shape
        F = x.size(1)
        dev = r.device
        ws = [t.detach().contiguous() for t in (wp2, bp2, wr0, br0, wr1, br1, wdr, bdr)]
        s, u, e, h0 = (torch.empty(N, D, dtype=torch.float32, device=dev) for _ in range(4))
        P = _lib.ptr
        _lib.call("gine_chain_fwd", P(r), P(x), P(ws[0]), P(ws[1]), float(members), P(ws[2]),
                  P(ws[3]), P(ws[4]), P(ws[5]), P(ws[6]), P(ws[7]), P(s), P(u), P(e), P(h0),
                  N, D, F, _lib.stream_handle(dev))
        ctx.save_for_backward(r, x, s, u, e, ws[0], ws[2], ws[4], ws[6])
        ctx.params = (wp2, bp2, wr0, br0, wr1, br1, wdr, bdr)
        ctx.members = float(members)
        return h0

    @staticmethod
    def backward(ctx, dh0):
        r, x, s, u, e, wp2, wr0, wr1, wdr = ctx.saved_tensors
        N, D = r.shape
        F = x.size(1)
        dev = r.device
        dh0 = dh0.contiguous()
        de, dt, ds, dr = (torch.empty(N, D, dtype=torch.float32, device=dev) for _ in range(4))
        floats = ctypes.c_size_t(0)
        _lib.call("gine_chain_bwd_slab_floats", N, D, F, ctypes.byref(floats))
        slab = torch.empty(floats.value, dtype=torch.float32, device=dev)
        p = ctx.params
        g = [grad_out(p[0], (D, D), dev), grad_out(p[1], (D,), dev),
             grad_out(p[2], (D, D), dev), grad_out(p[3], (D,), dev),
             grad_out(p[4], (D, D), dev), grad_out(p[5], (D,), dev),
             grad_out(p[6], (D, F + D), dev), grad_out(p[7], (D,), dev)]
        P = _lib.ptr
        _lib.call("gine_chain_bwd", P(dh0), P(x), P(r), P(s), P(u), P(e), P(wp2), P(wr0),
                  P(wr1), P(wdr), P(de), P(dt), P(ds), P(dr), None, None, None, ctx.members,
                  None, None, None, None, None, None, N, D, F, _lib.stream_handle(dev))
        members = ctx.members
        if gradbuf.deferrable(*g):
            _lib.call("gine_chain_wgrad", P(dh0), P(x), P(r), P(s), P(u), P(e), P(de),
                      P(dt), P(ds), P(slab), None, None, members, None, None, None, None,
                      None, None, N, D, F, _lib.stream_handle(dev))
            job = _lib.GradJob()
            _lib.call("gine_chain_wgrad_grad_job", N, D, F, P(slab), members, P(g[0]),
                      P(g[1]), P(g[2]), P(g[3]), P(g[4]), P(g[5]), P(g[6]), P(g[7]),
                      ctypes.byref(job))
            gradbuf.defer(job, dev, (slab,))
            return (dr, None, g[0], g[1], g[2], g[3], g[4], g[5], g[6], g[7], None)
        _lib.call("gine_chain_wgrad", P(dh0), P(x), P(r), P(s), P(u), P(e), P(de), P(dt),
                  P(ds), P(slab), P(g[0]), P(g[1]), members, P(g[2]), P(g[3]), P(g[4]),
                  P(g[5]), P(g[6]), P(g[7]), N, D, F, _lib.stream_handle(dev))
        return (dr, None, g[0], g[1], g[2], g[3], g[4], g[5], g[6], g[7], None)


class _ChainFolded2Fn(torch.autograd.Function):

    @staticmethod
    def forward(ctx, r, x, wp2, bp2, wr0, br0, wr1, br1, wdr, bdr, members, wfold):
        r = r.contiguous()
        x = x.contiguous()
        N, D = r.shape
        F = x.size(1)
        dev = r.device
        n1 = 2 * D * (F + D) + D
        wf1, wf2 = wfold[:n1], wfold[n1:]
        u, h0 = (torch.empty(N, D, dtype=torch.float32, device=dev) for _ in range(2))
        P = _lib.ptr
        _lib.call("gine_chain_fwd_folded2", P(r), P(x), P(wf1), P(wf2), P(u), P(h0), N, D, F,
                  _lib.stream_handle(dev))
        ws = [t.detach().contiguous() for t in (wp2, bp2, wr0, wr1, br1, wdr)]
        ctx.save_for_backward(r, x, u, wfold, *ws)
        ctx.params = (wp2, bp2, wr0, br0, wr1, br1, wdr, bdr)
        ctx.members = float(members)
        return h0

    @staticmethod
    def backward(ctx, dh0):
        r, x, u, wfold, wp2, bp2, wr0, wr1, br1, wdr = ctx.saved_tensors
        N, D = r.shape
        F = x.size(1)
        dev = r.device
        n1 = 2 * D * (F + D) + D
        wf1, wf2 = wfold[:n1], wfold[n1:]
        dh0 = dh0.contiguous()
        dt, dr = (torch.empty(N, D, dtype=torch.float32, device=dev) for _ in range(2))
        floats = ctypes.c_size_t(0)
        _lib.call("gine_chain_bwd_slab_floats", N, D, F, ctypes.byref(floats))
        slab = torch.empty(floats.value, dtype=torch.float32, device=dev)
        gf = torch.empty(D * (F + D) + D + D * D + D, dtype=torch.float32, device=dev)
        gfold, g2fold = gf[:D * (F + D) + D], gf[D * (F + D) + D:]
        p = ctx.params
        g = [grad_out(p[0], (D, D), dev), grad_out(p[1], (D,), dev),
             grad_out(p[2], (D, D), dev), grad_out(p[3], (D,), dev),
             grad_out(p[4], (D, D), dev), grad_out(p[5], (D,), dev),
             grad_out(p[6], (D, F + D), dev), grad_out(p[7], (D,), dev)]
        P = _lib.ptr
        stream = _lib.stream_handle(dev)
        _lib.call("gine_chain_bwd_folded2", P(dh0), P(u), P(wf1), P(wf2), P(dt), P(dr), N, D, F,
                  stream)
        ptrs = (P(gfold), P(wr1), P(br1), P(wdr), P(g[6]), P(g[7]), P(g[4]), P(g[5]),
                P(g2fold), P(wp2), P(bp2), P(wr0), P(g[2]), P(g[3]), P(g[0]), P(g[1]),
                ctx.members)

        def unfold(st):
            _lib.call("gine_chain_unfold_grads2", *ptrs, D, F, st)

        if gradbuf.deferrable(*g):
            _lib.call("gine_chain_wgrad_folded2", P(dh0), P(x), P(r), P(u), P(dt), P(slab), None,
                      None, N, D, F, stream)
            job = _lib.GradJob()
            _lib.call("gine_chain_wgrad_folded2_grad_job", N, D, F, P(slab), P(gfold),
                      P(g2fold), ctypes.byref(job))
            gradbuf.defer(job, dev, (slab, gf, wp2, bp2, wr0, wr1, br1, wdr), post=unfold)
        else:
            _lib.call("gine_chain_wgrad_folded2", P(dh0), P(x), P(r), P(u), P(dt), P(slab),
                      P(gfold), P(g2fold), N, D, F, stream)
            unfold(stream)
        return (dr, None, g[0], g[1], g[2], g[3], g[4], g[5], g[6], g[7], None, None)


FOLD = True


def chain(r: torch.Tensor, x: torch.Tensor, lins, members: int, wfold=None) -> torch.Tensor:
    p2, r0, r1, dr = lins
    if not FOLD:
        return _ChainFn.apply(r, x, p2.weight, p2.bias, r0.weight, r0.bias, r1.weight, r1.bias,
                              dr.weight, dr.bias, members)
    D, F = r.size(1), x.size(1)
    if wfold is None or wfold.numel() != 2 * D * (F + D) + D + D * D + D:
        raise ValueError(f"the folded chain needs wfold with [W' | b' | W'^T | Wf | bf] for "
                         f"D={D}, F={F}")
    return _ChainFolded2Fn.apply(r, x, p2.weight, p2.bias, r0.weight, r0.bias, r1.weight,
                                 r1.bias, dr.weight, dr.bias, members, wfold)
```

raincast-gnn_amd/raincast_gnn/deepset.py:

```python
from __future__ import annotations

import ctypes

import torch

from . import _lib
from . import gradbuf
from .gradbuf import grad_out

HIDDEN = (32, 64, 128, 256)
MAX_FEATURES = 64


def fusable(ens: torch.Tensor, weight: torch.Tensor, bias) -> bool:
    return (ens.is_cuda and ens.dim() == 3 and ens.dtype == torch.float32
            and weight.dtype == torch.float32 and bias is not None
            and weight.size(0) in HIDDEN and 0 < weight.size(1) <= MAX_FEATURES
            and ens.size(2) == weight.size(1) and ens.size(1) > 0
            and not ens.requires_grad)


class _PhiSumFn(torch.autograd.Function):
    @staticmethod
    def forward(ctx, ens, weight, bias, fold=None):
        ens = ens.contiguous()
        weight, bias = weight.contiguous(), bias.contiguous()
        N, M, Fdim = ens.shape
        H = weight.size(0)
        r = torch.empty(N, H, dtype=torch.float32, device=ens.device)
        mask = None
        if ctx.needs_input_grad[1] or ctx.needs_input_grad[2]:
            nbytes = ctypes.c_size_t(0)
            _lib.call("gine_deepset_mask_bytes", N, M, H, ctypes.byref(nbytes))
            mask = torch.empty(nbytes.value, dtype=torch.uint8, device=ens.device)
        ctx.save_for_backward(ens, mask)
        ctx.params = (weight, bias)
        ctx.hidden = H
        stream = _lib.stream_handle(ens.device)
        if fold is None:
            _lib.call("gine_deepset_fwd", _lib.ptr(ens), _lib.ptr(weight), _lib.ptr(bias),
                      _lib.ptr(r), _lib.ptr(mask), N, M, Fdim, H, stream)
            return r
        wr1, br1, wdr, bdr, wr0, br0, wp2, bp2 = (t.detach().contiguous() for t in fold)
        F = wdr.size(1) - H
        n1 = 2 * H * (F + H) + H
        P = _lib.ptr
        wfold = torch.empty(n1 + H * H + H, dtype=torch.float32, device=ens.device)
        _lib.call("gine_deepset_fwd_fold2", P(ens), P(weight), P(bias), P(r), P(mask), N, M,
                  Fdim, H, P(wr1), P(br1), P(wdr), P(bdr), P(wfold), F, P(wr0), P(br0),
                  P(wp2), P(bp2), P(wfold[n1:]), stream)
        ctx.mark_non_differentiable(wfold)
        ctx.set_materialize_grads(False)
        return r, wfold

    @staticmethod
    def backward(ctx, dr, *unused):
        ens, mask = ctx.saved_tensors
        if dr is None:
            return None, None, None, None
        N, M, Fdim = ens.shape
        H = ctx.hidden
        dr = dr.contiguous()
        parts = ctypes.c_int32(0)
        _lib.call("gine_deepset_bwd_num_partials", N, H, ctypes.byref(parts))
        slab = torch.empty(parts.value * (H * Fdim + H), dtype=torch.float32, device=dr.device)
        dw = grad_out(ctx.params[0], (H, Fdim), dr.device)
        db = grad_out(ctx.params[1], (H,), dr.device)
        defer = gradbuf.deferrable(dw, db)
        _lib.call("gine_deepset_bwd", _lib.ptr(ens), _lib.ptr(mask), _lib.ptr(dr),
                  _lib.ptr(slab), None if defer else _lib.ptr(dw),
                  None if defer else _lib.ptr(db), N, M, Fdim, H,
                  _lib.stream_handle(dr.device))
        if defer:
            job = _lib.GradJob()
            _lib.call("gine_deepset_bwd_grad_job", N, Fdim, H, _lib.ptr(slab), _lib.ptr(dw),
                      _lib.ptr(db), ctypes.byref(job))
            gradbuf.defer(job, dr.device, (slab,))
        return None, dw, db, None


def phi_sum(ens: torch.Tensor, lin1: torch.nn.Linear, fold=None):
    if fold is None:
        return _PhiSumFn.apply(ens, lin1.weight, lin1.bias)
    if len(fold) != 4:
        raise ValueError("fold = (rho[2], dim_red, rho[0], phi[2])")
    return _PhiSumFn.apply(ens, lin1.weight, lin1.bias,
                           tuple(t for m in fold for t in (m.weight, m.bias)))
```

raincast-gnn_amd/raincast_gnn/gradbuf.py:

```python
from __future__ import annotations

import threading
import weakref

import torch
from torch.utils.weak import WeakIdKeyDictionary

from . import _lib

_slots = WeakIdKeyDictionary()
_issued = WeakIdKeyDictionary()
_flats: list = []


def register(param: torch.Tensor, flat: torch.Tensor, offset: int) -> None:
    _slots[param] = (flat, offset)
    if not any(r() is flat for r in _flats):
        _flats.append(weakref.ref(flat))


def in_flat_buffer(t: torch.Tensor | None) -> bool:
    if t is None:
        return False
    p = t.data_ptr()
    for r in _flats:
        f = r()
        if f is not None and f.data_ptr() <= p < f.data_ptr() + 4 * f.numel():
            return True
    return False


def slice_of(param: torch.Tensor):
    slot = _slots.get(param)
    if slot is None:
        return None
    flat, off = slot
    return flat[off:off + param.numel()].view(param.shape)


def new_step(params) -> None:
    for p in params:
        _issued.pop(p, None)


def grad_out(param: torch.Tensor | None, shape=None, device=None) -> torch.Tensor:
    if param is not None and param.grad is None and param not in _issued:
        view = slice_of(param)
        if view is not None:
            _issued[param] = True
            return view if shape is None else view.view(shape)
    shp = param.shape if shape is None else shape
    dev = param.device if device is None else device
    return torch.empty(shp, dtype=torch.float32, device=dev)



BATCH_ENABLED = True
_pending: list = []
_pending_lock = threading.Lock()


def deferrable(*outs) -> bool:
    if not BATCH_ENABLED or not outs:
        return False
    if not all(in_flat_buffer(t) for t in outs if t is not None):
        return False
    return torch._C._current_graph_task_id() != -1


def defer(job: "_lib.GradJob", device: torch.device, keep_alive=(), post=None) -> None:
    stream = _lib.stream_handle(device)
    with _pending_lock:
        first = not _pending
        _pending.append((job, stream, tuple(keep_alive), post))
    if first:
        torch.autograd.Variable._execution_engine.queue_callback(flush)


def flush() -> None:
    with _pending_lock:
        items = list(_pending)
        _pending.clear()
    by_stream: dict = {}
    for job, stream, keep, post in items:
        by_stream.setdefault(stream, ([], []))
        by_stream[stream][0].append(job)
        if post is not None:
            by_stream[stream][1].append(post)
    for stream, (jobs, posts) in by_stream.items():
        for i in range(0, len(jobs), _lib.GRAD_MAX_JOBS):
            part = jobs[i:i + _lib.GRAD_MAX_JOBS]
            arr = (_lib.GradJob * len(part))(*part)
            _lib.call("gine_grad_finalize_batch", arr, len(part), stream)
        for post in posts:
            post(stream)


def mp_job(partials: torch.Tensor, rows: int, channels: int, eps_cols: int, dlw, dlb, deps):
    j = _lib.GradJob()
    j.kind = _lib.GRAD_JOB_MP
    j.src = partials.data_ptr()
    j.rows, j.channels, j.eps_cols = int(rows), int(channels), int(eps_cols)
    j.w[0], j.w[1], j.w[2] = dlw.data_ptr(), dlb.data_ptr(), deps.data_ptr()
    return j


_seeds: dict = {}


def loss_backward(loss: torch.Tensor) -> None:
    key = (loss.device, loss.dtype)
    one = _seeds.get(key)
    if one is None:
        if loss.is_cuda and torch.cuda.is_current_stream_capturing():
            loss.backward()
            return
        one = _seeds[key] = torch.ones((), dtype=loss.dtype, device=loss.device)
    loss.backward(one)


def is_unit_seed(g: torch.Tensor) -> bool:
    one = _seeds.get((g.device, g.dtype))
    return one is not None and g is one
```

raincast-gnn_amd/raincast_gnn/options.py:

```python
from __future__ import annotations

MP_FUSED = "1"
MP_WINDOW = "auto"
WINDOW_NODES = 128
ENGINE_IN_MP = True
BN_ACC = True
BN_ACC_BWD = True
LAYER_FWD = True
LAYER_WIN = False
LAYER_BWD = True
HEAD_FOLD = True
```

Baseline: 72170 graphs/s.

## Fuse chain weight-gradient blocks into deepset backward launch as rider blocks

The chain's deferred folded weight-gradient kernel is parked instead of launched, then runs as extra workgroups inside a combined deepset-backward kernel. Leading blocks do the chain wgrad tiles and the rest do the deepset walk. The aim is to drop one launch and let two under-filled kernels share the GPU concurrently. It also splits bias sums across row groups in the wgrad body. The cost is more Python bookkeeping to park and take riders, a fallback path, and a larger shared LDS footprint per block.

```diff
diff --git a/include/gine_hip.h b/include/gine_hip.h
--- a/include/gine_hip.h
+++ b/include/gine_hip.h
@@ -372,6 +372,14 @@
                              const float* bp2, const float* wr0, float* dwr0, float* dbr0,
                              float* dwp2, float* dbp2, float members, int32_t hidden,
                              int32_t in_features, void* stream);
+int gine_deepset_bwd_chain_wgrad_fits(int64_t num_nodes, int32_t hidden, int32_t in_features,
+                                      int32_t x_features, int32_t* ok);
+int gine_deepset_bwd_chain_wgrad(const float* ens, const uint16_t* mask, const float* dr,
+                                 float* slab, float* dw1, float* db1, int64_t num_nodes,
+                                 int32_t members, int32_t in_features, int32_t hidden,
+                                 const float* dh0, const float* x, const float* r,
+                                 const float* u, const float* dt, float* chain_slab,
+                                 int32_t x_features, void* stream);
 int gine_chain_fwd(const float* r, const float* x, const float* wp2, const float* bp2,
                    float bias_scale, const float* wr0, const float* br0, const float* wr1,
                    const float* br1, const float* wdr, const float* bdr, float* s, float* u,
diff --git a/raincast-gnn_amd/csrc/gine_chain.hip b/raincast-gnn_amd/csrc/gine_chain.hip
--- a/raincast-gnn_amd/csrc/gine_chain.hip
+++ b/raincast-gnn_amd/csrc/gine_chain.hip
@@ -1,6 +1,7 @@
 #include "gine_common.hpp"
 #include "gine_slab.hpp"
 #include "gine_wgrad.hpp"
+#include "gine_chainwg.hpp"
 #include "gine_chainfold.hpp"
 
 #include <algorithm>
@@ -315,56 +316,6 @@
   return GINE_OK;
 }
 
-template <int NZ>
-struct ChainWgradSrc {
-  static constexpr int kZ = NZ;
-  const float* p[NZ];
-  const float* q[NZ];
-  const float* x;
-  int D, F;
-  struct Raw {
-    float4 v;
-  };
-  struct Col {
-    float keep[4];
-  };
-  template <int Z> __device__ int i_dim(int) const { return Z == 0 ? F + D : D; }
-  template <int Z> __device__ Col p_col(int) const { return Col{{1.f, 1.f, 1.f, 1.f}}; }
-  template <int Z> __device__ Col q_col(int q4) const {
-    Col c{{1.f, 1.f, 1.f, 1.f}};
-    if constexpr (Z == 0) {
-#pragma unroll
-      for (int j = 0; j < 4; ++j) c.keep[j] = 4 * q4 + j < F + D ? 1.f : 0.f;
-    }
-    return c;
-  }
-  template <int Z> __device__ Raw p_load(int64_t n, int q4) const {
-    return Raw{reinterpret_cast<const float4*>(p[Z] + n * D)[q4]};
-  }
-  template <int Z> __device__ Raw q_load(int64_t n, int q4) const {
-    if constexpr (Z == 0) {
-      const int I = F + D;
-      float v[4];
-#pragma unroll
-      for (int j = 0; j < 4; ++j) {
-        const int c = min(4 * q4 + j, I - 1);
-        const float* src = c < F ? x + n * F + c : q[0] + n * D + (c - F);
-        v[j] = *src;
-      }
-      return Raw{make_float4(v[0], v[1], v[2], v[3])};
-    } else {
-      return Raw{reinterpret_cast<const float4*>(q[Z] + n * D)[q4]};
-    }
-  }
-  template <int Z> __device__ float4 p_xform(const Raw& r, const Col&) const { return r.v; }
-  template <int Z> __device__ float4 q_xform(const Raw& r, const Col& c) const {
-    if constexpr (Z == 0)
-      return make_float4(c.keep[0] != 0.f ? r.v.x : 0.f, c.keep[1] != 0.f ? r.v.y : 0.f,
-                         c.keep[2] != 0.f ? r.v.z : 0.f, c.keep[3] != 0.f ? r.v.w : 0.f);
-    return r.v;
-  }
-};
-
 struct ChainWgradOut {
   float* w[4];
   float* b[4];
@@ -380,24 +331,6 @@
     }
   }
 };
-
-struct ChainWgradShape {
-  WgPlan plan;
-  int nz;
-  int tiles;
-  size_t per;
-  size_t zstride() const { return per * plan.chunks; }
-  size_t slab_floats() const { return nz * zstride(); }
-};
-inline ChainWgradShape chain_wgrad_shape(int64_t N, int D, int F, int nz) {
-  const int to = (int)ceil_div(D, 64);
-  ChainWgradShape s;
-  s.nz = nz;
-  s.tiles = to * (int)ceil_div(F + D, kWgTI) + (nz - 1) * to * (int)ceil_div(D, kWgTI);
-  s.plan = wg_plan(N, D, F + D, nz, 64, s.tiles);
-  s.per = (size_t)D * (D + F) + D;
-  return s;
-}
 
 void chain_slab_job(const ChainWgradShape& sh, int D, int F, const float* slab, float bscale3,
                     float* const* w, float* const* b, gine_grad_job* job) {
@@ -417,8 +350,6 @@
     job->bscale[z] = z == 3 ? bscale3 : 1.0f;
   }
 }
-
-inline bool chain_dims_ok(int D, int F) { return (D == 64 || D == 128) && F >= 1 && F <= 64; }
 
 #define GINE_CHAIN_DISPATCH(D_, F_, CALL)                          \
   do {                                                             \
diff --git a/raincast-gnn_amd/csrc/gine_chainwg.hpp b/raincast-gnn_amd/csrc/gine_chainwg.hpp
--- /dev/null
+++ b/raincast-gnn_amd/csrc/gine_chainwg.hpp
@@ -0,0 +1,80 @@
+#pragma once
+
+#include "gine_common.hpp"
+#include "gine_wgrad.hpp"
+
+namespace gine {
+namespace {
+
+template <int NZ>
+struct ChainWgradSrc {
+  static constexpr int kZ = NZ;
+  const float* p[NZ];
+  const float* q[NZ];
+  const float* x;
+  int D, F;
+  struct Raw {
+    float4 v;
+  };
+  struct Col {
+    float keep[4];
+  };
+  template <int Z> __device__ int i_dim(int) const { return Z == 0 ? F + D : D; }
+  template <int Z> __device__ Col p_col(int) const { return Col{{1.f, 1.f, 1.f, 1.f}}; }
+  template <int Z> __device__ Col q_col(int q4) const {
+    Col c{{1.f, 1.f, 1.f, 1.f}};
+    if constexpr (Z == 0) {
+#pragma unroll
+      for (int j = 0; j < 4; ++j) c.keep[j] = 4 * q4 + j < F + D ? 1.f : 0.f;
+    }
+    return c;
+  }
+  template <int Z> __device__ Raw p_load(int64_t n, int q4) const {
+    return Raw{reinterpret_cast<const float4*>(p[Z] + n * D)[q4]};
+  }
+  template <int Z> __device__ Raw q_load(int64_t n, int q4) const {
+    if constexpr (Z == 0) {
+      const int I = F + D;
+      float v[4];
+#pragma unroll
+      for (int j = 0; j < 4; ++j) {
+        const int c = min(4 * q4 + j, I - 1);
+        const float* src = c < F ? x + n * F + c : q[0] + n * D + (c - F);
+        v[j] = *src;
+      }
+      return Raw{make_float4(v[0], v[1], v[2], v[3])};
+    } else {
+      return Raw{reinterpret_cast<const float4*>(q[Z] + n * D)[q4]};
+    }
+  }
+  template <int Z> __device__ float4 p_xform(const Raw& r, const Col&) const { return r.v; }
+  template <int Z> __device__ float4 q_xform(const Raw& r, const Col& c) const {
+    if constexpr (Z == 0)
+      return make_float4(c.keep[0] != 0.f ? r.v.x : 0.f, c.keep[1] != 0.f ? r.v.y : 0.f,
+                         c.keep[2] != 0.f ? r.v.z : 0.f, c.keep[3] != 0.f ? r.v.w : 0.f);
+    return r.v;
+  }
+};
+
+struct ChainWgradShape {
+  WgPlan plan;
+  int nz;
+  int tiles;
+  size_t per;
+  size_t zstride() const { return per * plan.chunks; }
+  size_t slab_floats() const { return nz * zstride(); }
+};
+inline ChainWgradShape chain_wgrad_shape(int64_t N, int D, int F, int nz) {
+  const int to = (int)ceil_div(D, 64);
+  ChainWgradShape s;
+  s.nz = nz;
+  s.tiles = to * (int)ceil_div(F + D, kWgTI) + (nz - 1) * to * (int)ceil_div(D, kWgTI);
+  s.plan = wg_plan(N, D, F + D, nz, 64, s.tiles);
+  s.per = (size_t)D * (D + F) + D;
+  return s;
+}
+
+inline bool chain_dims_ok(int D, int F) { return (D == 64 || D == 128) && F >= 1 && F <= 64; }
+
+}
+}
diff --git a/raincast-gnn_amd/csrc/gine_deepset.hip b/raincast-gnn_amd/csrc/gine_deepset.hip
--- a/raincast-gnn_amd/csrc/gine_deepset.hip
+++ b/raincast-gnn_amd/csrc/gine_deepset.hip
@@ -1,5 +1,6 @@
 #include "gine_common.hpp"
 #include "gine_chainfold.hpp"
+#include "gine_chainwg.hpp"
 #include "gine_bf16x3.hpp"
 
 #include <algorithm>
@@ -462,7 +463,7 @@
                                             const uint16_t* __restrict__ mask,
                                             const float* __restrict__ dr,
                                             float* __restrict__ slab, int64_t N, int M, int F,
-                                            int num_groups, float* s_lds) {
+                                            int num_groups, float* s_lds, int nb, int bw) {
   constexpr int NT = 2 * H;
   constexpr int KI = ds_bwd_ki(KP);
   using I = DsBwdImg<KI>;
@@ -480,14 +481,18 @@
     uint16_t* i0 = reinterpret_cast<uint16_t*>(s_e0);
     uint16_t* i1 = reinterpret_cast<uint16_t*>(s_e1);
     const int w = (KI - F) * I::RS;
-    for (int i = threadIdx.x; i < 3 * w; i += blockDim.x) {
+    for (int i = threadIdx.x; i < 3 * w; i += NT) {
       const int pl = i / w, e = F * I::RS + i % w;
       i0[pl * I::PLANE + e] = 0;
       i1[pl * I::PLANE + e] = 0;
     }
   } else {
-    zero_pad<KP>(s_e0, F);
-    zero_pad<KP>(s_e1, F);
+    constexpr int LD0 = KP + 4;
+    for (int i = threadIdx.x; i < 32 * (LD0 - F); i += NT) {
+      const int r = i / (LD0 - F), c = F + i % (LD0 - F);
+      s_e0[r * LD0 + c] = 0.f;
+      s_e1[r * LD0 + c] = 0.f;
+    }
   }
 
   floatx16 gw[NIF > 0 ? NIF : 1];
@@ -500,7 +505,7 @@
 
   Stager<NT, KP, G != 16, X3, KI, true> st;
   st.init(F, M, G);
-  const Groups gr(num_groups, gridDim.x);
+  const Groups gr(num_groups, nb, bw);
   const int GM = G * M, tpg = tiles_per_group(G, M);
   const float* my_dr = s_dr + G * h * H + col;
   int node = 0, rem = M;
@@ -583,7 +588,7 @@
     for (int it = 0; it < NIF; ++it) bad = bad || wave_any_nan(gw[it]);
     if (block_any(bad, reinterpret_cast<int*>(s_e0))) return false;
   }
-  float* out = slab + (size_t)blockIdx.x * ((size_t)H * F + H);
+  float* out = slab + (size_t)bw * ((size_t)H * F + H);
 #pragma unroll
   for (int it = 0; it < NIF; ++it) {
 #pragma unroll
@@ -620,10 +625,59 @@
                                                        int M, int F, int num_groups) {
   __shared__ __attribute__((aligned(16))) float s_lds[ds_bwd_lds_floats<H, KP, G>()];
 #if GINE_DS_BWD_BF16X3
-  if (ds_bwd_body<H, KP, G, true>(ens, mask, dr, slab, N, M, F, num_groups, s_lds)) return;
+  if (ds_bwd_body<H, KP, G, true>(ens, mask, dr, slab, N, M, F, num_groups, s_lds, gridDim.x,
+                                  blockIdx.x))
+    return;
   __syncthreads();
 #endif
-  ds_bwd_body<H, KP, G, false>(ens, mask, dr, slab, N, M, F, num_groups, s_lds);
+  ds_bwd_body<H, KP, G, false>(ens, mask, dr, slab, N, M, F, num_groups, s_lds, gridDim.x,
+                               blockIdx.x);
+}
+
+
+#ifndef GINE_DS_RIDER_WAVES
+#define GINE_DS_RIDER_WAVES 4
+#endif
+#ifndef GINE_DS_RIDER_MIN_NODES
+#define GINE_DS_RIDER_MIN_NODES 1
+#endif
+#ifndef GINE_DS_RIDER_MAX_NODES
+#define GINE_DS_RIDER_MAX_NODES (int64_t(1) << 30)
+#endif
+constexpr int kRiderWaves = GINE_DS_RIDER_WAVES;
+struct DsRider {
+  ChainWgradSrc<2> src;
+  int64_t R;
+  float* slab;
+  size_t zstride, cstride;
+  int D, I, rows_per_chunk, tiles, nblocks;
+};
+
+template <int H, int KP, int G>
+__global__ __launch_bounds__(64 * kRiderWaves) void k_deepset_bwd_rider(
+    const float* __restrict__ ens, const uint16_t* __restrict__ mask,
+    const float* __restrict__ dr, float* __restrict__ slab, int64_t N, int M, int F,
+    int num_groups, DsRider eng) {
+  static_assert(2 * H <= 64 * kRiderWaves, "the walk runs in the workgroup's first 2H threads");
+  constexpr size_t kWalk = sizeof(float) * ds_bwd_lds_floats<H, KP, G>();
+  constexpr size_t kEng = wg_lds_bytes<64>();
+  __shared__ __attribute__((aligned(16))) float s_lds[(kWalk > kEng ? kWalk : kEng) / sizeof(float)];
+  if ((int)blockIdx.x < eng.nblocks) {
+    const int e = xcd_remap(blockIdx.x, eng.nblocks);
+    wgrad_block<ChainWgradSrc<2>, 64, kRiderWaves, GINE_WG_BF16X3 != 0,
+                wg_bias_groups<64, kRiderWaves>()>(eng.src, eng.R, eng.D, eng.I, e / eng.tiles,
+                                                   e % eng.tiles, eng.rows_per_chunk,
+                                                   eng.zstride, eng.cstride, eng.slab, s_lds,
+                                                   s_lds + kWgRows * (64 + 4));
+    return;
+  }
+  if (2 * H < 64 * kRiderWaves && (int)threadIdx.x >= 2 * H) return;
+  const int nb = gridDim.x - eng.nblocks, bw = blockIdx.x - eng.nblocks;
+#if GINE_DS_BWD_BF16X3
+  if (ds_bwd_body<H, KP, G, true>(ens, mask, dr, slab, N, M, F, num_groups, s_lds, nb, bw)) return;
+  __syncthreads();
+#endif
+  ds_bwd_body<H, KP, G, false>(ens, mask, dr, slab, N, M, F, num_groups, s_lds, nb, bw);
 }
 
 __global__ __launch_bounds__(256) void k_deepset_slab_reduce(const float* __restrict__ slab,
@@ -831,6 +885,72 @@
   job->w[0] = dw1;
   job->b[0] = db1;
   job->bscale[0] = 1.0f;
+  return GINE_OK;
+}
+
+constexpr int64_t kRiderMinNodes = GINE_DS_RIDER_MIN_NODES;
+constexpr int64_t kRiderMaxNodes = GINE_DS_RIDER_MAX_NODES;
+inline bool rider_fits(int64_t N, int H, int F, int XF) {
+  if (H != 128 || F <= 0 || !chain_dims_ok(H, XF)) return false;
+  const int KP = pad_bwd(F);
+  if (KP < 0 || KP == 40 || KP == 64) return false;
+  return N >= kRiderMinNodes && N <= kRiderMaxNodes;
+}
+
+extern "C" int gine_deepset_bwd_chain_wgrad_fits(int64_t num_nodes, int32_t hidden,
+                                                 int32_t in_features, int32_t x_features,
+                                                 int32_t* ok) {
+  if (!ok || num_nodes < 0) return GINE_ERR_INVALID;
+  *ok = rider_fits(num_nodes, hidden, in_features, x_features) ? 1 : 0;
+  return GINE_OK;
+}
+
+extern "C" int gine_deepset_bwd_chain_wgrad(const float* ens, const uint16_t* mask,
+                                            const float* dr, float* slab, float* dw1, float* db1,
+                                            int64_t num_nodes, int32_t members,
+                                            int32_t in_features, int32_t hidden,
+                                            const float* dh0, const float* x, const float* r,
+                                            const float* u, const float* dt, float* chain_slab,
+                                            int32_t x_features, void* stream) {
+  if (num_nodes < 0 || members <= 0) return GINE_ERR_INVALID;
+  if (!rider_fits(num_nodes, hidden, in_features, x_features)) return GINE_ERR_DIM;
+  if (!ens || !mask || !dr || !slab) return GINE_ERR_INVALID;
+  if (!dh0 || !x || !r || !u || !dt || !chain_slab) return GINE_ERR_INVALID;
+  if (num_nodes * members >= (int64_t(1) << 31)) return GINE_ERR_TOO_LARGE;
+  const int KP = pad_bwd(in_features);
+  const int groups = num_groups(num_nodes, hidden);
+  const int grid = bwd_grid(num_nodes, hidden);
+  const int G = nodes_per_half(num_nodes, hidden);
+  const int D = hidden, XF = x_features;
+  const ChainWgradShape sh = chain_wgrad_shape(num_nodes, D, XF, 2);
+  DsRider eng{ChainWgradSrc<2>{{dh0, dt}, {u, r}, x, D, XF}, num_nodes, chain_slab,
+              sh.zstride(), sh.per, D, D + XF, sh.plan.rows_per_chunk, sh.tiles,
+              sh.plan.chunks * sh.tiles};
+  hipStream_t s = as_stream(stream);
+#define LAUNCH_RIDER_G(H_, KP_, G_)                                                          \
+  hipLaunchKernelGGL((k_deepset_bwd_rider<H_, KP_, G_>), dim3(eng.nblocks + grid),           \
+                     dim3(64 * kRiderWaves), 0, s, ens, mask, dr, slab, num_nodes, members,  \
+                     in_features, groups, eng)
+#define LAUNCH_RIDER(H_, KP_)                       \
+  do {                                              \
+    if (G == 4) LAUNCH_RIDER_G(H_, KP_, 4);         \
+    else if (G == 8) LAUNCH_RIDER_G(H_, KP_, 8);    \
+    else LAUNCH_RIDER_G(H_, KP_, 16);               \
+  } while (0)
+  switch (KP) {
+    case 16: LAUNCH_RIDER(128, 16); break;
+    case 32: LAUNCH_RIDER(128, 32); break;
+    case 36: LAUNCH_RIDER(128, 36); break;
+    default: LAUNCH_RIDER(128, 48); break;
+  }
+#undef LAUNCH_RIDER
+#undef LAUNCH_RIDER_G
+  GINE_LAUNCH_STATUS();
+  if (!dw1) return GINE_OK;
+  const int64_t per = (int64_t)hidden * in_features + hidden;
+  hipLaunchKernelGGL(k_deepset_slab_reduce, dim3((unsigned)ceil_div(per, 16)), dim3(256), 0, s,
+                     slab, grid, per, (int64_t)hidden * in_features, dw1, db1);
+  GINE_LAUNCH_STATUS();
   return GINE_OK;
 }
 
diff --git a/raincast-gnn_amd/csrc/gine_wgrad.hpp b/raincast-gnn_amd/csrc/gine_wgrad.hpp
--- a/raincast-gnn_amd/csrc/gine_wgrad.hpp
+++ b/raincast-gnn_amd/csrc/gine_wgrad.hpp
@@ -68,7 +68,10 @@
   return p;
 }
 
-template <class Src, int Z, int TO, int NW>
+template <int TO, int NW>
+constexpr int wg_bias_groups() { return (TO == 64 && NW == 4) ? 2 : 1; }
+
+template <class Src, int Z, int TO, int NW, int BG = 1>
 __device__ __forceinline__ void wgrad_body(const Src& src, int64_t R, int O, int I, int chunk,
                                            int tile, int rows_per_chunk, size_t zstride,
                                            size_t cstride, float* __restrict__ slab,
@@ -119,7 +122,8 @@
     for (int k = 0; k < NI; ++k)
 #pragma unroll
       for (int e = 0; e < 16; ++e) acc[j][k][e] = 0.f;
-  double bsum[4] = {0.0, 0.0, 0.0, 0.0};
+  static_assert(BG == 1 || BG == wg_bias_groups<TO, NW>(), "bias row groups");
+  double bsum[BG][4] = {};
 
   Raw rp[PITEMS]{}, rq[QITEMS]{};
   auto load_item = [&](int j, int64_t n0) {
@@ -148,10 +152,10 @@
       float4 v = src.template p_xform<Z>(rp[k], pc);
       if (n0 + r >= r_end || !p_ok) v = f4_zero();
       *reinterpret_cast<float4*>(&sP[r * LDP + 4 * pq]) = v;
-      bsum[0] += (double)v.x;
-      bsum[1] += (double)v.y;
-      bsum[2] += (double)v.z;
-      bsum[3] += (double)v.w;
+      bsum[k % BG][0] += (double)v.x;
+      bsum[k % BG][1] += (double)v.y;
+      bsum[k % BG][2] += (double)v.z;
+      bsum[k % BG][3] += (double)v.w;
     }
 #pragma unroll
     for (int k = 0; k < QITEMS; ++k) {
@@ -227,12 +231,14 @@
   if (bias_block) {
     double* sb = reinterpret_cast<double*>(sQ);
 #pragma unroll
-    for (int j = 0; j < 4; ++j) sb[pr * TO + 4 * pq + j] = bsum[j];
+    for (int gi = 0; gi < BG; ++gi)
+#pragma unroll
+      for (int j = 0; j < 4; ++j) sb[(pr + PG * gi) * TO + 4 * pq + j] = bsum[gi][j];
     __syncthreads();
     if ((int)threadIdx.x < TO && o0 + (int)threadIdx.x < O) {
       double t = 0.0;
 #pragma unroll 8
-      for (int g = 0; g < PG; ++g) t += sb[g * TO + threadIdx.x];
+      for (int g = 0; g < PG * BG; ++g) t += sb[g * TO + threadIdx.x];
       out[(size_t)O * I + o0 + threadIdx.x] = (float)t;
     }
   }
@@ -279,7 +285,7 @@
   return f;
 }
 
-template <class Src, int Z, int TO, int NW>
+template <class Src, int Z, int TO, int NW, int BG = 1>
 __device__ __forceinline__ void wgrad_body_x3(const Src& src, int64_t R, int O, int I,
                                               int chunk, int tile, int rows_per_chunk,
                                               size_t zstride, size_t cstride,
@@ -327,7 +333,8 @@
     for (int k = 0; k < NI; ++k)
 #pragma unroll
       for (int e = 0; e < 16; ++e) acc[j][k][e] = 0.f;
-  double bsum[4] = {0.0, 0.0, 0.0, 0.0};
+  static_assert(BG == 1 || BG == wg_bias_groups<TO, NW>(), "bias row groups");
+  double bsum[BG][4] = {};
 
   Raw rp[PITEMS]{}, rq[QITEMS]{};
   auto load_item = [&](int j, int64_t n0) {
@@ -356,10 +363,11 @@
         float4 v = src.template p_xform<Z>(rp[k], pc);
         if (n0 + r >= r_end || !p_ok) v = f4_zero();
         vp[k] = v;
-        bsum[0] += (double)v.x;
-        bsum[1] += (double)v.y;
-        bsum[2] += (double)v.z;
-        bsum[3] += (double)v.w;
+        constexpr int PB = PITEMS / BG;
+        bsum[k / PB][0] += (double)v.x;
+        bsum[k / PB][1] += (double)v.y;
+        bsum[k / PB][2] += (double)v.z;
+        bsum[k / PB][3] += (double)v.w;
       }
       wg_store_cols<TO, PITEMS>(imgP, pq, pr * PITEMS, vp);
 #pragma unroll
@@ -402,8 +410,8 @@
 #define GINE_WG_X3_NANCHECK 1
 #endif
   if (GINE_WG_X3_NANCHECK && block_any(bad, reinterpret_cast<int*>(imgP))) {
-    wgrad_body<Src, Z, TO, NW>(src, R, O, I, chunk, tile, rows_per_chunk, zstride, cstride,
-                               slab, sP, sQ);
+    wgrad_body<Src, Z, TO, NW, BG>(src, R, O, I, chunk, tile, rows_per_chunk, zstride,
+                                   cstride, slab, sP, sQ);
     return;
   }
 
@@ -424,28 +432,30 @@
   if (bias_block) {
     double* sb = reinterpret_cast<double*>(imgQ);
 #pragma unroll
-    for (int j = 0; j < 4; ++j) sb[pr * TO + 4 * pq + j] = bsum[j];
+    for (int gi = 0; gi < BG; ++gi)
+#pragma unroll
+      for (int j = 0; j < 4; ++j) sb[(pr * BG + gi) * TO + 4 * pq + j] = bsum[gi][j];
     __syncthreads();
     if ((int)threadIdx.x < TO && o0 + (int)threadIdx.x < O) {
       double t = 0.0;
 #pragma unroll 8
-      for (int g = 0; g < PG; ++g) t += sb[g * TO + threadIdx.x];
+      for (int g = 0; g < PG * BG; ++g) t += sb[g * TO + threadIdx.x];
       out[(size_t)O * I + o0 + threadIdx.x] = (float)t;
     }
   }
 }
 
-template <bool X3, class Src, int Z, int TO, int NW>
+template <bool X3, class Src, int Z, int TO, int NW, int BG = 1>
 __device__ __forceinline__ void wg_body(const Src& src, int64_t R, int O, int I, int chunk,
                                         int tile, int rows_per_chunk, size_t zstride,
                                         size_t cstride, float* __restrict__ slab, float* sP,
                                         float* sQ) {
   if constexpr (X3)
-    wgrad_body_x3<Src, Z, TO, NW>(src, R, O, I, chunk, tile, rows_per_chunk, zstride, cstride,
-                                  slab, sP, sQ);
+    wgrad_body_x3<Src, Z, TO, NW, BG>(src, R, O, I, chunk, tile, rows_per_chunk, zstride,
+                                      cstride, slab, sP, sQ);
   else
-    wgrad_body<Src, Z, TO, NW>(src, R, O, I, chunk, tile, rows_per_chunk, zstride, cstride,
-                               slab, sP, sQ);
+    wgrad_body<Src, Z, TO, NW, BG>(src, R, O, I, chunk, tile, rows_per_chunk, zstride,
+                                   cstride, slab, sP, sQ);
 }
 
 template <class Src, int Z>
@@ -453,23 +463,23 @@
   return (int)(ceil_div(O, TO) * ceil_div(src.template i_dim<Z>(I), kWgTI));
 }
 
-template <class Src, int TO, int NW, bool X3 = GINE_WG_BF16X3 != 0>
+template <class Src, int TO, int NW, bool X3 = GINE_WG_BF16X3 != 0, int BG = 1>
 __device__ __forceinline__ void wgrad_block(const Src& src, int64_t R, int O, int I, int chunk,
                                             int y, int rows_per_chunk, size_t zstride,
                                             size_t cstride, float* __restrict__ slab,
                                             float* sP, float* sQ) {
   const int t0 = wg_tiles<Src, 0>(src, O, I, TO);
   if (y < t0) {
-    wg_body<X3, Src, 0, TO, NW>(src, R, O, src.template i_dim<0>(I), chunk, y, rows_per_chunk,
-                               zstride, cstride, slab, sP, sQ);
+    wg_body<X3, Src, 0, TO, NW, BG>(src, R, O, src.template i_dim<0>(I), chunk, y,
+                                    rows_per_chunk, zstride, cstride, slab, sP, sQ);
     return;
   }
   y -= t0;
   if constexpr (Src::kZ > 1) {
     const int t1 = wg_tiles<Src, 1>(src, O, I, TO);
     if (y < t1) {
-      wg_body<X3, Src, 1, TO, NW>(src, R, O, src.template i_dim<1>(I), chunk, y,
-                                 rows_per_chunk, zstride, cstride, slab, sP, sQ);
+      wg_body<X3, Src, 1, TO, NW, BG>(src, R, O, src.template i_dim<1>(I), chunk, y,
+                                      rows_per_chunk, zstride, cstride, slab, sP, sQ);
       return;
     }
     y -= t1;
@@ -477,15 +487,15 @@
   if constexpr (Src::kZ > 2) {
     const int t2 = wg_tiles<Src, 2>(src, O, I, TO);
     if (y < t2) {
-      wg_body<X3, Src, 2, TO, NW>(src, R, O, src.template i_dim<2>(I), chunk, y,
-                                 rows_per_chunk, zstride, cstride, slab, sP, sQ);
+      wg_body<X3, Src, 2, TO, NW, BG>(src, R, O, src.template i_dim<2>(I), chunk, y,
+                                      rows_per_chunk, zstride, cstride, slab, sP, sQ);
       return;
     }
     y -= t2;
   }
   if constexpr (Src::kZ > 3) {
-    wg_body<X3, Src, 3, TO, NW>(src, R, O, src.template i_dim<3>(I), chunk, y, rows_per_chunk,
-                               zstride, cstride, slab, sP, sQ);
+    wg_body<X3, Src, 3, TO, NW, BG>(src, R, O, src.template i_dim<3>(I), chunk, y,
+                                    rows_per_chunk, zstride, cstride, slab, sP, sQ);
   }
 }
 
diff --git a/raincast-gnn_amd/raincast_gnn/_lib.py b/raincast-gnn_amd/raincast_gnn/_lib.py
--- a/raincast-gnn_amd/raincast_gnn/_lib.py
+++ b/raincast-gnn_amd/raincast_gnn/_lib.py
@@ -183,6 +183,9 @@
     "gine_chain_wgrad_folded2": [_c_void_p] * 8 + [_i64, _i32, _i32, _c_void_p],
     "gine_chain_wgrad_folded2_grad_job": [_i64, _i32, _i32] + [_c_void_p] * 3 + [_job_p],
     "gine_chain_unfold_grads2": [_c_void_p] * 16 + [_f32, _i32, _i32, _c_void_p],
+    "gine_deepset_bwd_chain_wgrad_fits": [_i64, _i32, _i32, _i32, ctypes.POINTER(_i32)],
+    "gine_deepset_bwd_chain_wgrad": [_c_void_p] * 6 + [_i64, _i32, _i32, _i32]
+                                    + [_c_void_p] * 6 + [_i32, _c_void_p],
 }
 
 EXPORTED_SYMBOLS = ("gine_abi_version", "gine_status_string") + tuple(_SIGNATURES)
diff --git a/raincast-gnn_amd/raincast_gnn/chain.py b/raincast-gnn_amd/raincast_gnn/chain.py
--- a/raincast-gnn_amd/raincast_gnn/chain.py
+++ b/raincast-gnn_amd/raincast_gnn/chain.py
@@ -4,11 +4,18 @@
 
 import torch
 
-from . import _lib, gradbuf
+from . import _lib, gradbuf, options
 from .gradbuf import grad_out
 
 HIDDEN = (64, 128)
 MAX_FEATURES = 64
+
+
+def rider_applies(N: int, D: int, ens_features: int, x_features: int) -> bool:
+    ok = ctypes.c_int32(0)
+    _lib.call("gine_deepset_bwd_chain_wgrad_fits", N, D, ens_features, x_features,
+              ctypes.byref(ok))
+    return bool(ok.value)
 
 
 def fusable(r: torch.Tensor, x: torch.Tensor, lins) -> bool:
@@ -135,12 +142,17 @@
             _lib.call("gine_chain_unfold_grads2", *ptrs, D, F, st)
 
         if gradbuf.deferrable(*g):
-            _lib.call("gine_chain_wgrad_folded2", P(dh0), P(x), P(r), P(u), P(dt), P(slab), None,
-                      None, N, D, F, stream)
+            ride = options.DS_RIDER and rider_applies(N, D, 1, F)
+            if not ride:
+                _lib.call("gine_chain_wgrad_folded2", P(dh0), P(x), P(r), P(u), P(dt), P(slab),
+                          None, None, N, D, F, stream)
             job = _lib.GradJob()
             _lib.call("gine_chain_wgrad_folded2_grad_job", N, D, F, P(slab), P(gfold),
                       P(g2fold), ctypes.byref(job))
             gradbuf.defer(job, dev, (slab, gf, wp2, bp2, wr0, wr1, br1, wdr), post=unfold)
+            if ride:
+                gradbuf.park_rider(dev, gradbuf.Rider((dh0, x, r, u, dt, slab), dr.data_ptr(),
+                                                      N, D, F, stream))
         else:
             _lib.call("gine_chain_wgrad_folded2", P(dh0), P(x), P(r), P(u), P(dt), P(slab),
                       P(gfold), P(g2fold), N, D, F, stream)
diff --git a/raincast-gnn_amd/raincast_gnn/deepset.py b/raincast-gnn_amd/raincast_gnn/deepset.py
--- a/raincast-gnn_amd/raincast_gnn/deepset.py
+++ b/raincast-gnn_amd/raincast_gnn/deepset.py
@@ -6,6 +6,7 @@
 
 from . import _lib
 from . import gradbuf
+from .chain import rider_applies
 from .gradbuf import grad_out
 
 HIDDEN = (32, 64, 128, 256)
@@ -67,10 +68,22 @@
         dw = grad_out(ctx.params[0], (H, Fdim), dr.device)
         db = grad_out(ctx.params[1], (H,), dr.device)
         defer = gradbuf.deferrable(dw, db)
-        _lib.call("gine_deepset_bwd", _lib.ptr(ens), _lib.ptr(mask), _lib.ptr(dr),
-                  _lib.ptr(slab), None if defer else _lib.ptr(dw),
-                  None if defer else _lib.ptr(db), N, M, Fdim, H,
-                  _lib.stream_handle(dr.device))
+        stream = _lib.stream_handle(dr.device)
+        rider = gradbuf.take_rider(dr.device, dr.data_ptr(), N, stream)
+        if rider is not None and not (rider.D == H
+                                      and rider_applies(N, H, Fdim, rider.F)):
+            gradbuf.park_rider(dr.device, rider)
+            rider = None
+        if rider is not None:
+            P = _lib.ptr
+            dh0, x, r, u, dt, cslab = rider.tensors
+            _lib.call("gine_deepset_bwd_chain_wgrad", P(ens), P(mask), P(dr), P(slab),
+                      None if defer else P(dw), None if defer else P(db), N, M, Fdim, H,
+                      P(dh0), P(x), P(r), P(u), P(dt), P(cslab), rider.F, stream)
+        else:
+            _lib.call("gine_deepset_bwd", _lib.ptr(ens), _lib.ptr(mask), _lib.ptr(dr),
+                      _lib.ptr(slab), None if defer else _lib.ptr(dw),
+                      None if defer else _lib.ptr(db), N, M, Fdim, H, stream)
         if defer:
             job = _lib.GradJob()
             _lib.call("gine_deepset_bwd_grad_job", N, Fdim, H, _lib.ptr(slab), _lib.ptr(dw),
diff --git a/raincast-gnn_amd/raincast_gnn/gradbuf.py b/raincast-gnn_amd/raincast_gnn/gradbuf.py
--- a/raincast-gnn_amd/raincast_gnn/gradbuf.py
+++ b/raincast-gnn_amd/raincast_gnn/gradbuf.py
@@ -77,10 +77,54 @@
         torch.autograd.Variable._execution_engine.queue_callback(flush)
 
 
+class Rider:
+    __slots__ = ("tensors", "dr_ptr", "N", "D", "F", "stream", "task")
+
+    def __init__(self, tensors, dr_ptr, N, D, F, stream):
+        self.tensors, self.dr_ptr, self.N, self.D, self.F = tuple(tensors), dr_ptr, N, D, F
+        self.stream = stream
+        self.task = torch._C._current_graph_task_id()
+
+    def launch_alone(self) -> None:
+        P = _lib.ptr
+        dh0, x, r, u, dt, slab = self.tensors
+        _lib.call("gine_chain_wgrad_folded2", P(dh0), P(x), P(r), P(u), P(dt), P(slab), None,
+                  None, self.N, self.D, self.F, self.stream)
+
+
+_riders: dict = {}
+
+
+def park_rider(device: torch.device, rider: Rider) -> None:
+    with _pending_lock:
+        old = _riders.pop(device, None)
+        _riders[device] = rider
+    if old is not None:
+        old.launch_alone()
+
+
+def take_rider(device: torch.device, dr_ptr: int, N: int, stream) -> Rider | None:
+    with _pending_lock:
+        r = _riders.get(device)
+        if (r is None or r.dr_ptr != dr_ptr or r.N != N or r.stream != stream
+                or r.task != torch._C._current_graph_task_id()):
+            return None
+        return _riders.pop(device)
+
+
+def rider_parked(device: torch.device) -> bool:
+    with _pending_lock:
+        return device in _riders
+
+
 def flush() -> None:
     with _pending_lock:
         items = list(_pending)
         _pending.clear()
+        riders = list(_riders.values())
+        _riders.clear()
+    for rider in riders:
+        rider.launch_alone()
     by_stream: dict = {}
     for job, stream, keep, post in items:
         by_stream.setdefault(stream, ([], []))
diff --git a/raincast-gnn_amd/raincast_gnn/options.py b/raincast-gnn_amd/raincast_gnn/options.py
--- a/raincast-gnn_amd/raincast_gnn/options.py
+++ b/raincast-gnn_amd/raincast_gnn/options.py
@@ -10,3 +10,4 @@
 LAYER_WIN = False
 LAYER_BWD = True
 HEAD_FOLD = True
+DS_RIDER = True
```

Measured after the change: 72670 graphs/s (median of 6 runs). Within noise of the previous version (+0.7%).
